# tingiskhan/pyfilter

Measured on AMD Instinct MI355X. Metric: particle-steps/sec (batch x particles x T), 1M-particle APF, higher is better.
Workload: dtype f32; 1 GPU; apf_lgo_1m: APF + lgo proposal, systematic resampling, N=1048576 particles x B=1 filters per GPU, T=250, state dim 1; parallelism=single GPU

## Files before the change

### include/pf_amd.h

```cpp
#ifndef PF_AMD_H
#define PF_AMD_H

#include <stddef.h>
#include <stdint.h>

#ifdef __cplusplus
extern "C" {
#endif

#define PF_ABI_VERSION 4

#define PF_OK 0
#define PF_EINVAL (-1)
#define PF_EWORKSPACE (-2)
#define PF_EUNSUPPORTED (-3)

#define PF_F32 0
#define PF_F64 1

#define PF_HID_LINEAR 0
#define PF_HID_SINE_EM 1
#define PF_HID_VERHULST_EM 2
#define PF_HID_LORENZ63_EM 3
#define PF_HID_OU 4
// ... 55 lines not shown

int pf_pre_weight(const pf_model* model, int proposal, const void* x, const void* y, int64_t y_rows, void* out,
                  int64_t N, int64_t B, int dtype, void* stream);

int pf_sample_and_weight(const pf_model* model, int proposal, int weigh, const void* x, const void* y,
                         int64_t y_rows, const void* z, uint64_t seed, uint32_t step, void* x_out, void* w_out,
                         int64_t N, int64_t B, int dtype, void* stream);

#define PF_NESTED_MAX 256
int pf_nested_sample_and_weight(const pf_model* model, int num_samples, const void* x, const void* y, int64_t y_rows,
                                const void* z, const void* v, uint64_t seed, uint32_t step, void* x_out, void* w_out,
                                int32_t* pick_out, int64_t N, int64_t B, int dtype, void* stream);

int pf_forecast_workspace_bytes(int64_t N, int64_t B, int steps, size_t* bytes);
int pf_forecast(const pf_model* model, int steps, const void* x, const void* W, const void* z, const void* e, uint64_t seed,
                void* x_mean, void* x_var, void* y_mean, void* y_var, void* x_path, void* y_path, void* ws, size_t ws_bytes,
                int64_t N, int64_t B, int dtype, void* stream);

int pf_initial_sample(const double* m0, const double* s0, const void* z, uint64_t seed, void* x, int64_t N,
                      int64_t B, int64_t D, int dtype, void* stream);

int pf_initial_sample_cols(const void* m0, int64_t m0_stride_b, int64_t m0_stride_d, const void* s0, int64_t s0_stride_b,
                           int64_t s0_stride_d, const void* z, uint64_t seed, void* x, int64_t N, int64_t B, int64_t D,
                           int dtype, void* stream);

int pf_observed_flags(const void* y, int64_t steps, int64_t row_elems, int dtype, uint8_t* out, void* stream);

int pf_theta_ess(const void* logw, int64_t rows, int64_t B, int dtype, void* out, void* stream);

#define PF_THETA_MAXP 8
#define PF_PRIOR_NORMAL 0
#define PF_PRIOR_LOGNORMAL 1
#define PF_PRIOR_EXPONENTIAL 2
#define PF_PRIOR_GAMMA 3
#define PF_PRIOR_HALFNORMAL 4
#define PF_PRIOR_BETA 5
#define PF_PRIOR_UNIFORM 6
typedef struct pf_theta_priors {
    int32_t P;
    int32_t kind[PF_THETA_MAXP];
    double a[PF_THETA_MAXP], b[PF_THETA_MAXP];
} pf_theta_priors;

int pf_theta_fit(const void* values, const void* logw, int64_t B, int32_t P, double scale, int dtype, void* mean, void* chol,
                 void* stream);

int pf_theta_propose(const pf_theta_priors* priors, const void* mean, const void* chol, const void* eps, int64_t B, int dtype,
                     void* u_out, void* const* x_out, void* prior_out, void* stream);

int pf_theta_accept(const void* u_cur, const void* u_star, const void* mean_f, const void* chol_f, const void* mean_r,
                    const void* chol_r, const void* prior_cur, const void* prior_star, const void* ll_cur, const void* ll_star,
                    const void* unif, int64_t B, int32_t P, int dtype, void* log_acc, uint8_t* accepted, void* rate, void* stream);

int pf_theta_path(const void* w0, const void* ll, int64_t n, int64_t B, int dtype, void* w_path, void* stats, void* host_rows,
                  uint64_t seq, const int32_t* status, void* stream);

int pf_theta_step(void* w, const void* ll, int64_t B, int dtype, void* stats, void* host_slot, uint64_t seq, void* acc,
                  const int32_t* status, void* stream);

int pf_host_alloc(size_t bytes, void** out);
int pf_host_free(void* p);

int pf_theta_resample(const void* logw, int64_t B, double u, int dtype, int64_t* ancestors, void* cdf_scratch, void* stream);

#define PF_JITTER_NONSHRINKING 0
#define PF_JITTER_SHRINKING 1
#define PF_JITTER_LIUWEST 2
#define PF_JITTER_CONSTANT 3
#define PF_JITTER_MAXB 8192

int pf_jitter_fit(const void* values, const void* logw, int64_t B, int32_t P, int32_t kind, double par, const void* scale,
                  double min_std, double bw_lo, double bw_hi, int dtype, double* fit, void* mean, void* scale_out, void* stream);

int pf_jitter_apply(const pf_theta_priors* priors, const void* values, const int64_t* ancestors, const double* fit, int64_t B,
                    int32_t kind, double par, double bw_lo, double bw_hi, int32_t discrete, const void* eps, const void* select,
                    uint64_t seed, uint64_t counter, int dtype, void* u_out, void* const* x_out, void* stream);

#define PF_ROUTE_AUTO 0
#define PF_ROUTE_PER_STEP 1
#define PF_ROUTE_COLUMN_GENERIC 2
#define PF_ROUTE_CLUSTER 3
#define PF_ROUTE_CLUSTER_ALWAYS 4
#define PF_ROUTE_CLUSTER_SPREAD 5
typedef struct pf_run_hints {
    int32_t route;
    int32_t column_max_n;
    int32_t tile_target;
    int32_t ancestor_search;
    int32_t resume;
    int32_t prepare_next;
    int32_t cluster_generation;
    int32_t cluster_patience;
} pf_run_hints;

typedef struct pf_filter_args {
    uint64_t struct_size;
    pf_model model;
    int32_t filter;
    int32_t proposal;
    int32_t resampler;
    int32_t dtype;
    int64_t N, B;
    double ess_threshold;
    uint64_t seed;
    void* x[2];
    void* logw[2];
    int32_t* anc;
    void* cdf;
    void* pos;
    const void* y;
    int64_t y_rows;
    const uint8_t* observed;
    const void* z_tape;
    const void* u_tape;
    void* means;
    void* vars;
    void* ll_steps;
    void* ll_total;
    int32_t* step_counter;
    void* ws;
    size_t ws_bytes;
    const uint8_t* observed_dev;
    int64_t ring;
    const void* user_loc;
    const void* user_scale;
    int64_t user_scale_per_column;
    double user_dt;
    int32_t* status;
    pf_run_hints hints;
} pf_filter_args;

int pf_filter_run(const pf_filter_args* args, int64_t t0, int64_t n_steps, int finalize, void* stream);

int pf_filter_observe(const pf_filter_args* args, int64_t t0, int64_t n_steps, int finalize, void* w, const void* ll, void* stats,
                      void* host_slot, uint64_t seq, void* acc, void* stream);

int pf_filter_graph_create(const pf_filter_args* args, int64_t t0, int64_t n_steps, int finalize, void* stream,
                           void** handle);
int pf_filter_graph_launch(void* handle, void* stream);
int pf_filter_graph_destroy(void* handle);

int pf_filter_run_timed(const pf_filter_args* args, int64_t t0, int64_t n_steps, int finalize, void* stream,
                        float* kernel_ms);


int pf_smooth_fixed_lag(const void* x_hist, const int32_t* anc_hist, void* out, int64_t S, int64_t N, int64_t B,
                        int64_t D, int dtype, void* stream);

int pf_smooth_ffbs(const pf_model* model, const void* x_hist, const void* logw_hist, const void* x_last, const void* u,
                   uint64_t seed, void* out, int64_t S, int64_t N, int64_t B, int dtype, void* stream);


int pf_debug_draw_normals(uint64_t seed, uint32_t step0, int64_t n_steps, void* out, int64_t N, int64_t B, int64_t D,
                          int dtype, void* stream);

int pf_debug_launch_trace(int32_t* out, int max_records);

#ifdef __cplusplus
}
#endif
#endif
```

### pyfilter_amd/_lib.py

```python
import ctypes as C
import os
from typing import Optional

import torch

_HERE = os.path.dirname(os.path.abspath(__file__))
LIB_PATH = os.path.join(_HERE, "libpfamd.so")

PF_F32, PF_F64 = 0, 1
HID_LINEAR, HID_SINE_EM, HID_VERHULST_EM, HID_LORENZ63_EM, HID_OU, HID_USER_AFFINE, HID_LINEAR_MAT = 0, 1, 2, 3, 4, 5, 6
OBS_LINEAR, OBS_SV = 0, 1
PROP_BOOTSTRAP, PROP_LGO = 0, 1
FILTER_SISR, FILTER_APF = 0, 1
RESAMPLE_SYSTEMATIC, RESAMPLE_MULTINOMIAL = 0, 1
MAX_D = 3
MAX_O = 3
LIN_MAX_D = 8
LIN_MAX_O = 8
NESTED_MAX = 256

EXPORTS = (
    "pf_version", "pf_abi_version", "pf_error_string", "pf_workspace_bytes", "pf_normalize", "pf_systematic", "pf_systematic_cdf_free", "pf_systematic_logw",
    "pf_multinomial", "pf_gather", "pf_loglik", "pf_moments", "pf_pre_weight", "pf_sample_and_weight",
    "pf_initial_sample", "pf_filter_run", "pf_filter_run_timed", "pf_filter_graph_create", "pf_filter_graph_launch",
    "pf_filter_graph_destroy", "pf_columns_gather", "pf_columns_exchange", "pf_debug_draw_normals", "pf_debug_launch_trace",
    "pf_smooth_fixed_lag", "pf_smooth_ffbs", "pf_observed_flags", "pf_theta_ess", "pf_theta_fit", "pf_theta_propose",
    "pf_theta_accept", "pf_theta_path", "pf_theta_resample", "pf_initial_sample_cols", "pf_theta_step", "pf_host_alloc",
    "pf_host_free", "pf_filter_observe", "pf_jitter_fit", "pf_jitter_apply", "pf_nested_sample_and_weight",
    "pf_forecast", "pf_forecast_workspace_bytes",
)


THETA_MAXP = 8
JITTER_NONSHRINKING, JITTER_SHRINKING, JITTER_LIUWEST, JITTER_CONSTANT = 0, 1, 2, 3
JITTER_MAXB = 8192


class PfThetaPriors(C.Structure):
    _fields_ = [("P", C.c_int32), ("kind", C.c_int32 * THETA_MAXP), ("a", C.c_double * THETA_MAXP), ("b", C.c_double * THETA_MAXP)]


class PfModel(C.Structure):
    _fields_ = [
        ("hid_kind", C.c_int32), ("obs_kind", C.c_int32), ("dim", C.c_int32), ("obs_dim", C.c_int32),
        ("dt", C.c_double), ("inc_scale", C.c_double), ("params", C.c_void_p),
    ]


ABI_VERSION = 4


class PfRunHints(C.Structure):
    _fields_ = [("route", C.c_int32), ("column_max_n", C.c_int32), ("tile_target", C.c_int32), ("ancestor_search", C.c_int32),
                ("resume", C.c_int32), ("prepare_next", C.c_int32), ("cluster_generation", C.c_int32), ("cluster_patience", C.c_int32)]


class PfFilterArgs(C.Structure):

    _fields_ = [
        ("struct_size", C.c_uint64),
        ("model", PfModel),
        ("filter", C.c_int32), ("proposal", C.c_int32), ("resampler", C.c_int32), ("dtype", C.c_int32),
        ("N", C.c_int64), ("B", C.c_int64),
        ("ess_threshold", C.c_double),
        ("seed", C.c_uint64),
        ("x", C.c_void_p * 2), ("logw", C.c_void_p * 2),
        ("anc", C.c_void_p), ("cdf", C.c_void_p), ("pos", C.c_void_p),
        ("y", C.c_void_p), ("y_rows", C.c_int64), ("observed", C.c_void_p),
        ("z_tape", C.c_void_p), ("u_tape", C.c_void_p),
        ("means", C.c_void_p), ("vars", C.c_void_p), ("ll_steps", C.c_void_p), ("ll_total", C.c_void_p),
        ("step_counter", C.c_void_p),
        ("ws", C.c_void_p), ("ws_bytes", C.c_size_t),
        ("observed_dev", C.c_void_p),
        ("ring", C.c_int64),
        ("user_loc", C.c_void_p), ("user_scale", C.c_void_p), ("user_scale_per_column", C.c_int64),
        ("user_dt", C.c_double),
        ("status", C.c_void_p),
        ("hints", PfRunHints),
    ]

    def __init__(self, *args, **kwargs):
        super().__init__(*args, **kwargs)
        self.struct_size = C.sizeof(PfFilterArgs)


_lib = None


class PfAmdError(RuntimeError):
    pass


def load() -> C.CDLL:
    global _lib
    if _lib is not None:
        return _lib
    path = LIB_PATH
    if not os.path.exists(path):
        raise PfAmdError(
            f"{path} not found: build it with `python -c 'import __graft_entry__ as g; g.build()'` "
            "(hipcc --offload-arch=gfx950).  pyfilter_amd has no CPU / eager fallback."
        )
    lib = C.CDLL(path)
    lib.pf_version.restype = C.c_char_p
    lib.pf_error_string.restype = C.c_char_p
    lib.pf_error_string.argtypes = [C.c_int]
    vp, i64, i32, u64, u32, sz = C.c_void_p, C.c_int64, C.c_int, C.c_uint64, C.c_uint32, C.c_size_t
    lib.pf_workspace_bytes.argtypes = [i64, i64, i64, C.POINTER(sz)]
    lib.pf_normalize.argtypes = [vp, vp, vp, vp, i64, i64, i32, vp, sz, vp]
    lib.pf_systematic.argtypes = [vp, vp, i32, vp, vp, vp, i64, i64, i32, vp, sz, vp]
    lib.pf_systematic_logw.argtypes = [vp, vp, i32, vp, vp, vp, i64, i64, i32, vp, sz, vp]
    lib.pf_systematic_cdf_free.argtypes = [i64, i64, i32, i32, C.POINTER(C.c_int)]
    lib.pf_multinomial.argtypes = [vp, vp, u64, u32, vp, vp, vp, i64, i64, i32, vp, sz, vp]
    lib.pf_gather.argtypes = [vp, vp, vp, vp, i64, i64, i64, i32, vp]
    lib.pf_loglik.argtypes = [vp, vp, vp, i64, i64, i32, vp, sz, vp]
    lib.pf_columns_gather.argtypes = [vp, vp, vp, i64, i64, i64, i32, vp]
    lib.pf_columns_exchange.argtypes = [vp, vp, vp, i64, i64, i64, i32, vp]
    lib.pf_moments.argtypes = [vp, vp, vp, vp, i64, i64, i64, i32, vp, sz, vp]
    lib.pf_pre_weight.argtypes = [C.POINTER(PfModel), i32, vp, vp, i64, vp, i64, i64, i32, vp]
    lib.pf_sample_and_weight.argtypes = [C.POINTER(PfModel), i32, i32, vp, vp, i64, vp, u64, u32, vp, vp, i64, i64, i32, vp]
    lib.pf_nested_sample_and_weight.argtypes = [C.POINTER(PfModel), i32, vp, vp, i64, vp, vp, u64, u32, vp, vp, vp, i64, i64, i32, vp]
    lib.pf_forecast_workspace_bytes.argtypes = [i64, i64, i32, C.POINTER(sz)]
    lib.pf_forecast.argtypes = [C.POINTER(PfModel), i32, vp, vp, vp, vp, u64, vp, vp, vp, vp, vp, vp, vp, sz, i64, i64, i32, vp]
    lib.pf_initial_sample.argtypes = [C.POINTER(C.c_double), C.POINTER(C.c_double), vp, u64, vp, i64, i64, i64, i32, vp]
    lib.pf_filter_run.argtypes = [C.POINTER(PfFilterArgs), i64, i64, i32, vp]
    lib.pf_filter_run_timed.argtypes = [C.POINTER(PfFilterArgs), i64, i64, i32, vp, C.POINTER(C.c_float)]
    lib.pf_filter_graph_create.argtypes = [C.POINTER(PfFilterArgs), i64, i64, i32, vp, C.POINTER(vp)]
    lib.pf_filter_graph_launch.argtypes = [vp, vp]
    lib.pf_filter_graph_destroy.argtypes = [vp]
    lib.pf_smooth_fixed_lag.argtypes = [vp, vp, vp, i64, i64, i64, i64, i32, vp]
    lib.pf_smooth_ffbs.argtypes = [C.POINTER(PfModel), vp, vp, vp, vp, u64, vp, i64, i64, i64, i32, vp]
    lib.pf_observed_flags.argtypes = [vp, i64, i64, i32, vp, vp]
    lib.pf_theta_ess.argtypes = [vp, i64, i64, i32, vp, vp]
    lib.pf_theta_path.argtypes = [vp, vp, i64, i64, i32, vp, vp, vp, u64, vp, vp]
    lib.pf_theta_resample.argtypes = [vp, i64, C.c_double, i32, vp, vp, vp]
    lib.pf_theta_step.argtypes = [vp, vp, i64, i32, vp, vp, u64, vp, vp, vp]
    lib.pf_filter_observe.argtypes = [C.POINTER(PfFilterArgs), i64, i64, i32, vp, vp, vp, vp, u64, vp, vp]
    lib.pf_host_alloc.argtypes = [sz, C.POINTER(vp)]
    lib.pf_host_free.argtypes = [vp]
    lib.pf_initial_sample_cols.argtypes = [vp, i64, i64, vp, i64, i64, vp, u64, vp, i64, i64, i64, i32, vp]
    lib.pf_theta_fit.argtypes = [vp, vp, i64, i32, C.c_double, i32, vp, vp, vp]
    lib.pf_theta_propose.argtypes = [C.POINTER(PfThetaPriors), vp, vp, vp, i64, i32, vp, C.POINTER(vp), vp, vp]
    lib.pf_theta_accept.argtypes = [vp] * 11 + [i64, i32, i32, vp, vp, vp, vp]
    dbl = C.c_double
    lib.pf_jitter_fit.argtypes = [vp, vp, i64, i32, i32, dbl, vp, dbl, dbl, dbl, i32, vp, vp, vp, vp]
    lib.pf_jitter_apply.argtypes = [C.POINTER(PfThetaPriors), vp, vp, vp, i64, i32, dbl, dbl, dbl, i32, vp, vp, u64, u64, i32, vp,
                                    C.POINTER(vp), vp]
    lib.pf_debug_draw_normals.argtypes = [u64, u32, i64, vp, i64, i64, i64, i32, vp]
    lib.pf_debug_launch_trace.argtypes = [C.POINTER(C.c_int32), i32]
    for name in EXPORTS:
        fn = getattr(lib, name)
        if name not in ("pf_version", "pf_error_string"):
            fn.restype = C.c_int
    if lib.pf_abi_version() != ABI_VERSION:
        raise PfAmdError(f"{path} implements ABI {lib.pf_abi_version()}, this package speaks ABI {ABI_VERSION}: rebuild it "
                         "(python -c 'import __graft_entry__ as g; g.build()')")
    _lib = lib
    return lib


def version() -> str:
    return load().pf_version().decode()


def check(rc: int, what: str):
    if rc != 0:
        raise PfAmdError(f"{what} failed: {load().pf_error_string(rc).decode()} (code {rc})")


def dtype_code(dtype: torch.dtype) -> int:
    if dtype == torch.float32:
        return PF_F32
    if dtype == torch.float64:
        return PF_F64
    raise PfAmdError(f"unsupported dtype {dtype}: the HIP kernels compute in float32 or float64")


def require_gpu(*tensors: Optional[torch.Tensor]):
    for t in tensors:
        if t is not None and not t.is_cuda:
            raise PfAmdError(
                "pyfilter_amd runs on MI355X only: got a CPU tensor (there is no CPU fallback; move the model / data "
                "to 'cuda')."
            )


def ptr(t: Optional[torch.Tensor]) -> Optional[int]:
    return None if t is None else t.data_ptr()


def stream_ptr() -> int:
    return torch._C._cuda_getCurrentRawStream(torch._C._cuda_getDevice())


_ws_cache = {}


def workspace(n: int, b: int, device: torch.device) -> torch.Tensor:
    key = (n, b, device.index, stream_ptr())
    ws = _ws_cache.get(key)
    nbytes = C.c_size_t(0)
    if ws is None:
        check(load().pf_workspace_bytes(n, b, 1, C.byref(nbytes)), "pf_workspace_bytes")
        ws = torch.empty(nbytes.value, dtype=torch.uint8, device=device)
        if len(_ws_cache) > 64:
            _ws_cache.clear()
        _ws_cache[key] = ws
    return ws


def new_workspace(n: int, b: int, device: torch.device) -> torch.Tensor:
    nbytes = C.c_size_t(0)
    check(load().pf_workspace_bytes(n, b, MAX_D, C.byref(nbytes)), "pf_workspace_bytes")
    return torch.zeros(nbytes.value, dtype=torch.uint8, device=device)
```

### pyfilter_amd/csrc/pf_fused.hpp

```cpp
#pragma once

namespace pf {

#define PF_STEP_B blockIdx.x
#define PF_STEP_K blockIdx.y

#ifdef PF_DEVTOOLS
#define PF_CUT(a, n) ((a).debug_cut == (n))
#define PF_STAMP(a, slot)                                                                       \
    do {                                                                                        \
        if ((a).debug_cut < 0 && !(a).finalize_only && PF_STEP_K == (unsigned)(-(a).debug_cut - 1) &&  \
            PF_STEP_B == 0 && threadIdx.x == 0)                                                 \
            (a).dbg[slot] = (unsigned long long)clock64();                                      \
    } while (0)
#else
#define PF_CUT(a, n) false
#ifdef PF_ISA_MARKS
#define PF_STAMP(a, slot) asm volatile("; PF_MARK " #slot)
#else
#define PF_STAMP(a, slot) do { } while (0)
#endif
#endif

template <typename T> struct FusedArgs {
    ModelDesc md;
    const T* params;
    int filter, proposal, resampler;
    Geom g;
    double thr_abs;
    double logN;
    T rcN;
    uint64_t seed;
    const uint64_t* seed_dev;
    T* x[2];
    T* logw[2];
    int32_t* anc;
    const int32_t* anc_prev;
    T* cdf;
    T* pos;
    const T* y;
    int y_rows;
    const T* z_tape;
    const T* u_tape;
    const T* user_loc;
    const T* user_scale;
    int user_scale_percol;
    T user_dt;
    T* means;
    T* vars;
    T* ll_steps;
    T* ll_total;
    double* part;
    int64_t part_stride;
    ColStat* stat;
    int32_t* poison;
    T* cpack;
    double* piv0;
    double* ctab;
    int64_t ctab_stride;
    int t0;
    int step;
    int obs;
    int obs_next;
    const uint8_t* obs_dev;
    __device__ __forceinline__ bool y_informative() const {
        const T* yr = y + (int64_t)step * md.obs_dim;
        bool any = false;
        for (int o = 0; o < md.obs_dim; ++o) any = any || !(yr[o] != yr[o]);
        return any;
    }
    __device__ __forceinline__ bool is_obs() const { return obs >= 0 ? obs != 0 : (obs == -1 ? obs_dev[step] != 0 : y_informative()); }
    __device__ __forceinline__ bool is_obs_next() const { return obs_next >= 0 ? obs_next != 0 : obs_dev[step + 1] != 0; }
    int finalize_only;
    int book_inline;
    unsigned kmap;
    __device__ __forceinline__ int tile_of_row(unsigned y) const {
        return (int)(((y & (kmap & 0xffu)) << ((kmap >> 8) & 0xffu)) + (y >> ((kmap >> 16) & 0xffu)));
    }
    unsigned long long* dbg;
    __device__ __forceinline__ const double* part_r() const { return part + (int64_t)(step & 1) * part_stride; }
    __device__ __forceinline__ double* part_w(int state) const { return part + (int64_t)(state & 1) * part_stride; }
    __device__ __forceinline__ const double* ctab_r(int b) const {
        return ctab + (int64_t)(step & 1) * ctab_stride + (int64_t)b * g.tiles * g.rounds_per_tile * PF_NWAVES * 2;
    }
    __device__ __forceinline__ double* ctab_w(int state, int b) const {
        return ctab + (int64_t)(state & 1) * ctab_stride + (int64_t)b * g.tiles * g.rounds_per_tile * PF_NWAVES * 2;
    }
    template <int D> __device__ __forceinline__ T pivot(int q, int b, int d) const {
        return (q - 2 >= t0) ? means[((int64_t)(q - 2) * g.B + b) * D + d] : (T)piv0[(int64_t)b * PF_MAXD + d];
    }
    int debug_cut;
    int keep_state;
};

template <typename T, int D>
__device__ __forceinline__ void load_col_params(const FusedArgs<T>& a, int b, int step, bool with_y, ColParams<T, D>& cp,
                                                int late = 0) {
    const int O = a.md.obs_dim;
    const int NP = 4 * D + O * D + 2 * O;
    cp.load(a.params + (int64_t)b * NP + late, O,
            with_y ? a.y + ((int64_t)step * a.y_rows + (a.y_rows == 1 ? 0 : b)) * O + late : nullptr);
}

template <typename T, int D, bool WQ = true> struct PartialAcc {
    T m1, m2;
    T s1, s2, q1;
    T mx[D], mxx[D];
    double es;
    bool poison;
    __device__ __forceinline__ void init() {
        m1 = m2 = -Lim<T>::inf();
        s1 = s2 = q1 = T(0);
        es = 0.0;
#pragma unroll
        for (int d = 0; d < D; ++d) mx[d] = mxx[d] = T(0);
        poison = false;
    }
    template <int VEC>
    __device__ __forceinline__ void push_round(const T (&lw)[VEC], const T (&x)[D][VEC], bool pre_on, const T (&pre)[VEC],
                                               const T (&piv)[D], T (&e_out)[VEC]) {
        T m = lw[0];
#pragma unroll
        for (int j = 1; j < VEC; ++j) m = (lw[j] > m) ? lw[j] : m;
        if (m > m1) {
            const T rs = (m1 == -Lim<T>::inf()) ? T(0) : pf_exp_w(m1 - m);
            s1 *= rs;
            if constexpr (WQ) q1 *= rs * rs;
#pragma unroll
            for (int d = 0; d < D; ++d) {
                mx[d] *= rs;
                mxx[d] *= rs;
            }
            m1 = m;
        }
#pragma unroll
        for (int j = 0; j < VEC; ++j) {
            T e = (lw[j] == -Lim<T>::inf()) ? T(0) : pf_exp_w(lw[j] - m1);
            if (lw[j] != lw[j]) e = lw[j];
            e_out[j] = e;
            s1 += e;
            if constexpr (WQ) q1 += e * e;
#pragma unroll
            for (int d = 0; d < D; ++d) {
                const T xd = x[d][j] - piv[d];
                mx[d] += e * xd;
                mxx[d] += e * xd * xd;
            }
        }
        if (pre_on) {
            T rw[VEC];
#pragma unroll
            for (int j = 0; j < VEC; ++j) {
                if (is_nan_or_posinf(pre[j])) poison = true;
                rw[j] = sanitize_logw(pre[j] + lw[j]);
            }
            T mm = rw[0];
#pragma unroll
            for (int j = 1; j < VEC; ++j) mm = (rw[j] > mm) ? rw[j] : mm;
            if (mm > m2) {
                s2 *= (m2 == -Lim<T>::inf()) ? T(0) : pf_exp_w(m2 - mm);
                m2 = mm;
            }
#pragma unroll
            for (int j = 0; j < VEC; ++j) {
                const T e = (rw[j] == -Lim<T>::inf()) ? T(0) : pf_exp_w(rw[j] - m2);
                e_out[j] = e;
                s2 += e;
            }
        }
    }
    template <bool WITH_ES, typename FB, typename FA>
    __device__ __forceinline__ void finish(double* part, int b, int k, int B, int tiles, bool pre_on, double* red, T* redm,
                                           int32_t* poison_slot, T& M1_out, T& M2_out, T& F1_out, T& F2_out, FB&& before, FA&& after) {
        const int lane = threadIdx.x & 63, wid = threadIdx.x >> 6;
        const T w1 = wave_max<T>(m1), w2 = wave_max<T>(m2);
        if (lane == 0) {
            redm[wid] = w1;
// ... 520 lines not shown
    double mv[2 * D];
    ColPartials<true, 2 * D> p1;
    ColPartials<false, 0> p2;
    load_col_partials<true, 2 * D>(a.part_r(), stride, cb, g.tiles, PQ_M1, PQ_S1, PQ_MX, p1);
    if (two) load_col_partials<false, 0>(a.part_r(), stride, cb, g.tiles, PQ_M2, PQ_S2, 0, p2);
    const ColSums c1 = column_sums<T, true, false, 2 * D>(p1, g.tiles, nullptr, nullptr, redm, red, mv);
    ColSums c2{0.0, 1.0, 0.0};
    if (two) c2 = column_sums<T, false, false>(p2, g.tiles, nullptr, nullptr, redm, red);
    const double lse_w = c1.M + log(c1.S);
    const double ess = c1.S * c1.S / c1.Q;
    bool resample = apf ? obs : (ess < a.thr_abs);
    if (a.finalize_only) resample = false;
    if (threadIdx.x == 0) {
#pragma unroll
        for (int d = 0; d < D; ++d) {
            const double dm = mv[d] / c1.S;
            double var = mv[D + d] / c1.S - dm * dm;
            if (var < 0.0) var = 0.0;
            a.means[((int64_t)step * g.B + b) * D + d] = (T)(piv[d] + dm);
            a.vars[((int64_t)step * g.B + b) * D + d] = (T)var;
        }
        if (step > 0 && !st.ll_done) {
            double ll = 0.0;
            if (st.prev_observed) {
                ll = lse_w - st.base_lse;
                if (poisoned) ll = __builtin_nan("");
            }
            a.poison[pslot * g.B + b] = 0;
            a.ll_steps[(int64_t)(step - 1) * g.B + b] = (T)ll;
            a.ll_total[b] = (T)(ll_tot + ll);
        }
        st.lse_w = lse_w;
        if (!a.finalize_only) st.resample = resample ? 1 : 0;
        st.ll_done = a.finalize_only ? 1 : 0;
        if (!a.finalize_only) {
            st.prev_observed = obs ? 1 : 0;
            st.base_lse = apf ? a.logN - ((c2.M + log(c2.S)) - lse_w) : (resample ? a.logN : lse_w);
        }
        a.stat[b] = st;
    }
}

template <typename T, int D>
__global__ __launch_bounds__(PF_BLOCK) void k_fused_book(FusedArgs<T> a) {
    __shared__ double red[(2 + 2 * D) * PF_NWAVES];
    __shared__ double redm[PF_NWAVES];
    column_bookkeeping<T, D>(a, blockIdx.y, red, redm);
}

#define PF_WAVES_D1_GENERIC 4
#define PF_WAVES_D1_MN 3
#define PF_WAVES_DN_A 3
template <typename T, int D, int MODE, int PROP, bool FAST, int SPEC, bool MULTI> struct StepWaves {
    static constexpr int value = sizeof(T) != 4 ? 1
                                 : (D == 1 && MODE == 1 && MULTI) ? PF_WAVES_D1_MN
                                 : D == 1     ? (FAST ? 4 : PF_WAVES_D1_GENERIC)
                                 : PROP == PF_PROP_LGO ? 2
                                 : (MODE == 1 || SPEC == 2) ? PF_WAVES_DN_A
                                 : 3;
};
template <typename T, int D, int VEC> struct StepShared {
    static constexpr int WIN = SearchWin<T, VEC>::WIN;
    static constexpr bool XWIN = (sizeof(T) * D <= 8);
    T* win;
    T* xwin;
    int* sh_j0;
    int* sh_cl;
    int* sh_wm;
    double* red;
    double* reds;
    T* redm;
    double* ptl;
    double* ftl;
    int* sh_plan;
    double* crec;
};
template <typename T> struct StepPlan {
    int j0, kt0;
    T ub;
    double offE, invE;
    bool resample;
    bool have_z0;
};
template <typename T, int D, int VEC, int MODE, int SPEC, bool EARLY_Z, bool MULTI>
__device__ __forceinline__ StepPlan<T> step_prologue(const FusedArgs<T>& a, const StepShared<T, D, VEC>& sh, T (&z0)[VEC][D]) {
    const Geom& g = a.g;
    const int b = PF_STEP_B, k = a.tile_of_row(PF_STEP_K);
    const int step = a.step;
    const bool obs = SPEC ? true : a.is_obs();
    const bool apf = SPEC ? (SPEC == 1) : (a.filter == PF_FILTER_APF);
    const bool two = apf && obs;
    StepPlan<T> pl{0, 0, T(0), 0.0, 0.0, false, false};
    PF_STAMP(a, 0);
#ifdef PF_DEVTOOLS
    if (a.debug_cut < 0 && threadIdx.x == 0 && b == 0 && (k % 128) == 0 && k / 128 < 8) a.dbg[16 + k / 128] = wall_clock64();
#endif
    if (apf && !obs) return pl;
    constexpr bool multinomial = MODE == 1;
    const uint64_t seed = a.seed + (a.seed_dev ? *a.seed_dev : 0ull);
    const T u_taped = (!multinomial && a.u_tape) ? a.u_tape[(int64_t)step * g.B + b] : T(0);
    const int64_t stride = (int64_t)g.B * g.tiles;
    const int64_t cb = (int64_t)b * g.tiles;
    double* const redm_d = sh.red + 2 * PF_NWAVES;
    T e0[1] = {T(0)};
    if constexpr (multinomial) {
        T tail[1];
        draw_exponentials<T, 1>(seed, PF_STREAM_MULTINOMIAL, (uint32_t)step, (uint64_t)((int64_t)g.B * g.N + b), tail);
        spacing_table(a.part_r(), stride, cb, g.tiles, (double)tail[0], sh.ptl, sh.reds);
        pl.offE = sh.ptl[k];
        pl.invE = 1.0 / sh.ptl[g.tiles + 1];
        draw_exponentials<T, 1>(seed, PF_STREAM_MULTINOMIAL, (uint32_t)step, (uint64_t)((int64_t)b * g.N + (int64_t)k * g.tile_elems), e0);
    }
    ColPartials<true, 0> p1;
    ColPartials<false, 0> p2;
    constexpr bool SHORT = MULTI;
    const bool one_tile = SHORT && g.tiles == 1 && a.debug_cut != 77;
    double m1 = 0.0, s1 = 0.0, q1 = 0.0;
    if (one_tile) {
        const double* part = a.part_r();
        m1 = part[(two ? PQ_M2 : PQ_M1) * stride + cb];
        s1 = part[(two ? PQ_S2 : PQ_S1) * stride + cb];
        q1 = two ? 0.0 : part[PQ_Q1 * stride + cb];
    }
    const bool few_tiles = SHORT && !one_tile && g.tiles <= PF_WAVE && a.debug_cut != 79;
    if (!one_tile && !few_tiles) {
        if (two) load_col_partials<false, 0>(a.part_r(), stride, cb, g.tiles, PQ_M2, PQ_S2, 0, p2);
        else load_col_partials<true, 0>(a.part_r(), stride, cb, g.tiles, PQ_M1, PQ_S1, 0, p1);
    }
    if (EARLY_Z && (SPEC || !a.z_tape)) {
        const int64_t i0 = (int64_t)k * g.tile_elems + threadIdx.x * VEC;
        if (i0 < g.N) draw_normals<T, D, VEC>(seed, PF_STREAM_NORMAL, (uint32_t)step, (uint64_t)((int64_t)b * g.N + i0), z0);
        pl.have_z0 = true;
    }
    if (one_tile) {
        if (two) {
            column_sums_one_tile<T, false>(m1, s1, q1, sh.ptl, sh.ftl);
            pl.resample = true;
        } else {
            const ColSums c = column_sums_one_tile<T, true>(m1, s1, q1, sh.ptl, sh.ftl);
            pl.resample = c.S * c.S / c.Q < a.thr_abs;
        }
    } else if (few_tiles) {
        if (two) {
            column_sums_wave<T, false>(a.part_r(), stride, cb, g.tiles, PQ_M2, PQ_S2, sh.ptl, sh.ftl);
            pl.resample = true;
        } else {
            const ColSums c = column_sums_wave<T, true>(a.part_r(), stride, cb, g.tiles, PQ_M1, PQ_S1, sh.ptl, sh.ftl);
            pl.resample = c.S * c.S / c.Q < a.thr_abs;
        }
    } else if (two) {
        column_sums<T, false, true>(p2, g.tiles, sh.ptl, sh.ftl, redm_d, sh.red);
        pl.resample = true;
    } else {
        const ColSums c = column_sums<T, true, true>(p1, g.tiles, sh.ptl, sh.ftl, redm_d, sh.red);
        pl.resample = c.S * c.S / c.Q < a.thr_abs;
    }
    PF_STAMP(a, 1);
    if (!pl.resample) return pl;
    const double* ptl = sh.ptl;
    T p;
    if constexpr (multinomial) {
        p = (T)((pl.offE + (double)e0[0]) * pl.invE);
    } else {
        pl.ub = a.u_tape ? u_taped : uniform_draw<T>(seed, PF_STREAM_UNIFORM, (uint32_t)step, (uint64_t)b);
        p = grid_position<T>((int64_t)k * g.tile_elems, pl.ub, T(g.N));
    }
    if (one_tile && a.debug_cut != 78) {
        pl.j0 = 0;
        pl.kt0 = 0;
        return pl;
    }
    if (threadIdx.x < PF_WAVE) {
        const int lane = threadIdx.x;
        int lo = 0, hi = g.tiles - 1;
        while (lo < hi) {
            const int len = hi - lo + 1;
            const int st = (len + PF_WAVE - 1) / PF_WAVE;
            int probe = lo + (lane + 1) * st - 1;
            if (probe > hi) probe = hi;
            const bool ge = (probe >= g.tiles - 1) || !((T)ptl[probe + 1] < p);
            const unsigned long long bal = __ballot(ge);
            const int f = bal ? __ffsll((long long)bal) - 1 : PF_WAVE - 1;
            int nhi = lo + (f + 1) * st - 1;
            if (nhi > hi) nhi = hi;
            lo = lo + f * st;
            if (lo > nhi) lo = nhi;
            hi = nhi;
        }
        const int kt = lo;
        const double Pk = ptl[kt], Pn = ptl[kt + 1], fk = sh.ftl[kt];
        const int64_t first = (int64_t)kt * g.tile_elems;
        const int64_t last = (first + g.tile_elems < g.N ? first + g.tile_elems : g.N) - 1;
        const T* l_col = ((step & 1) ? a.pos : a.cdf) + (int64_t)b * g.N;
        const int64_t len = last + 1 - first;
        auto cdf_at = [&](int64_t q) -> T {
            if constexpr (MULTI) {
                const double* cg = a.ctab_r(b) + 2 * (q / (PF_WAVE * VEC));
                return cdf_from_local<T>(l_col[q], cg[0], cg[1], Pk, fk, Pn, q == last, q == g.N - 1);
            } else {
                return cdf_from_local<T>(l_col[q], Pk, fk, Pn, q == last, q == g.N - 1);
            }
        };
        int64_t res;
        bool found;
        {
            float fr = (float)((double)p - Pk) * __builtin_amdgcn_rcpf((float)(Pn - Pk));
            fr = __builtin_fminf(__builtin_fmaxf(fr, 0.0f), 1.0f);
            int64_t g0 = first + (int64_t)(fr * (float)len) - (PF_WAVE / 2) * PF_PROBE_STEP;
            const int64_t g0max = last - (PF_WAVE - 1) * PF_PROBE_STEP;
            if (g0 > g0max) g0 = g0max;
            if (g0 < first) g0 = first;
            int64_t q = g0 + (int64_t)lane * PF_PROBE_STEP;
            if (q > last) q = last;
            const unsigned long long bal = __ballot(cdf_at(q) >= p);
            const int f = bal ? __ffsll((long long)bal) - 1 : 0;
            found = bal != 0 && (f > 0 || g0 == first);
            res = f > 0 ? g0 + (int64_t)(f - 1) * PF_PROBE_STEP + 1 : first;
        }
        if (!found) {
            const int64_t st = (len + PF_WAVE - 1) / PF_WAVE;
            int64_t probe = first + (lane + 1) * st - 1;
            if (probe > last) probe = last;
            const unsigned long long bal = __ballot(cdf_at(probe) >= p);
            const int f = bal ? __ffsll((long long)bal) - 1 : PF_WAVE - 1;
            res = first + (int64_t)f * st;
            if (res > last) res = last;
        }
        if (lane == 0) {
            sh.sh_plan[0] = (int)res;
            sh.sh_plan[1] = kt;
        }
    }
    __syncthreads();
    pl.j0 = sh.sh_plan[0];
    pl.kt0 = sh.sh_plan[1];
    PF_STAMP(a, 2);
    return pl;
}
template <typename T, int D, int VEC, int MODE, int PROP, bool FAST, int SPEC, int MK, bool RS, bool MULTI>
__device__ __forceinline__ void step_body(const FusedArgs<T>& a, const StepShared<T, D, VEC>& sh, const StepPlan<T>& pl,
                                          const T (&z0)[VEC][D]) {
    const int proposal = (PROP >= 0) ? PROP : a.proposal;
    ModelDesc md = a.md;
    if constexpr (!FAST && MK == 1) { md.hid_kind = PF_HID_VERHULST_EM; md.obs_kind = PF_OBS_SV; md.obs_dim = 1; }
    if constexpr (!FAST && MK == 4) { md.hid_kind = PF_HID_LORENZ63_EM; md.obs_kind = PF_OBS_LINEAR; }
    constexpr bool USER = !FAST && MK == 3;
    constexpr int WIN = StepShared<T, D, VEC>::WIN;
    constexpr int V1 = (MODE == 0) ? 1 : VEC;
    constexpr int STAGED = PF_BLOCK * (VEC + V1);
    constexpr bool XWIN = StepShared<T, D, VEC>::XWIN;
    T* const win = sh.win;
    T* const xwin = sh.xwin;
    int& sh_j0 = *sh.sh_j0;
    int* const sh_cl = sh.sh_cl;
    int* const sh_wm = sh.sh_wm;
    double* const red = sh.red;
    double* const reds = sh.reds;
    T* const redm = sh.redm;
    int* hd = reinterpret_cast<int*>(win);
    const Geom& g = a.g;
    const int b = PF_STEP_B, k = a.tile_of_row(PF_STEP_K);
    const int tid = threadIdx.x;
    const int step = a.step;
    const int slot = step & 1;
    const bool obs = SPEC ? true : a.is_obs();
    const bool apf = SPEC ? (SPEC == 1) : (a.filter == PF_FILTER_APF);
    constexpr bool resample = RS;
    constexpr bool multinomial = MODE == 1;
    const bool windowed = resample;
    const bool pre_next = SPEC ? (SPEC == 1) : (a.is_obs_next() && apf);
    const int N = (int)g.N;
    PF_STAMP(a, 8);
    if (PF_CUT(a, 1)) return;

    int j0 = pl.j0;
    int kt0 = pl.kt0;
    const double offE = pl.offE, invE = pl.invE;
    double carryE = 0.0;
    const uint64_t seed = a.seed + (a.seed_dev ? *a.seed_dev : 0ull);
    const T* z_step = (!SPEC && a.z_tape) ? a.z_tape + (int64_t)step * D * g.B * g.N : nullptr;

    ColParams<T, D> cp;
    ColConsts<T, D> cc;
    FastCol<T> fc;
    if constexpr (!FAST && D > 1) {
        load_col_params<T, D>(a, b, step, obs, cp);
        if (pre_next) cp.load_next(a.y + ((int64_t)(step + 1) * a.y_rows + (a.y_rows == 1 ? 0 : b)) * a.md.obs_dim);
    }
    const T ub = pl.ub;

    const T* x_in = a.x[slot];
    const T* lw_in = a.logw[slot] + (int64_t)b * g.N;
#ifdef PF_DEVTOOLS
    T* lw_out = a.logw[slot ^ 1] + (int64_t)b * g.N;
    int32_t* anc_col = a.anc + (int64_t)b * g.N;
#endif
    const T* cdf_col = ((step & 1) ? a.pos : a.cdf) + (int64_t)b * g.N;
    const int64_t base = (int64_t)k * g.tile_elems;
    const T nT = T(N);
    const T rcN = a.rcN;
    const bool pow2 = (N & (N - 1)) == 0;

    bool poison = false;
    PartialAcc<T, D, SPEC != 1> acc;
    acc.init();
    PF_STAMP(a, 9);
    const double* ptab_col = sh.ptl;
    const double* ftab_col = sh.ftl;
    CdfView<T> view;
    view.L = cdf_col;
    view.ptab = ptab_col;
    view.ftab = ftab_col;
    const double* const ct_col = MULTI ? a.ctab_r(b) : nullptr;
    view.ct = ct_col;
    view.chunk_elems = PF_WAVE * VEC;
    view.N = N;
    view.tile_elems = g.tile_elems;
    view.tiles = g.tiles;

    T e_rw[VEC];
    T rwn[VEC];
#pragma unroll
    for (int j = 0; j < VEC; ++j) {
        e_rw[j] = T(0);
        rwn[j] = -Lim<T>::inf();
    }
    const bool scan_next = !apf || pre_next;
    constexpr bool single = !MULTI;
    const bool use_lds = g.rounds_per_tile * PF_NWAVES <= PF_LDS_CHUNKS;
    double* const ct_tile = a.ctab_w(step + 1, b) + 2 * (int64_t)k * g.rounds_per_tile * PF_NWAVES;
    T* const l_next = ((step & 1) ? a.cdf : a.pos) + (int64_t)b * g.N;
    int rk = 0;
    for (int r = 0; r < g.rounds_per_tile; ++r) {
        const int64_t r0 = base + (int64_t)r * g.round_elems;
        if (r0 >= g.N) break;
        const int64_t i0 = r0 + tid * VEC;
        const bool on = i0 < g.N;
        if (MODE == 0 && windowed) {
            int zero[VEC];
#pragma unroll
            for (int j = 0; j < VEC; ++j) zero[j] = 0;
            if (VEC == 1) hd[tid] = 0; else store_vec<int, VEC>(hd + tid * VEC, zero);
        }
        T pv[VEC];
        if (multinomial && windowed) {
            T ev[VEC];
            double incl[VEC], local = 0.0, total;
            if (on) draw_exponentials<T, VEC>(seed, PF_STREAM_MULTINOMIAL, (uint32_t)step, (uint64_t)((int64_t)b * g.N + i0), ev);
#pragma unroll
            for (int j = 0; j < VEC; ++j) {
                local += on ? (double)ev[j] : 0.0;
                incl[j] = local;
            }
            const double excl = block_scan_excl(local, reds, total);
#pragma unroll
            for (int j = 0; j < VEC; ++j) pv[j] = (T)((offE + carryE + excl + incl[j]) * invE);
            carryE += total;
        }

        const int ws = j0 - (j0 % VEC);
        T c0[VEC], c1[V1], xa[D][VEC], xb[D][V1];
        const int ja = ws + tid * VEC, jb = ws + PF_BLOCK * VEC + tid * V1;
        const bool ina = windowed && ja < N, inb = windowed && jb < N;
        if (ina) {
            if (VEC == 1) c0[0] = cdf_col[ja]; else load_vec<T, VEC>(cdf_col + ja, c0);
            if (XWIN) {
#pragma unroll
                for (int d = 0; d < D; ++d) {
                    const T* xc = x_in + ((int64_t)d * g.B + b) * g.N + ja;
                    if (VEC == 1) xa[d][0] = xc[0]; else load_vec<T, VEC>(xc, xa[d]);
                }
            }
        }
        if (inb) {
            if (V1 == 1) c1[0] = cdf_col[jb]; else load_vec<T, V1>(cdf_col + jb, c1);
            if (XWIN) {
#pragma unroll
                for (int d = 0; d < D; ++d) {
                    const T* xc = x_in + ((int64_t)d * g.B + b) * g.N + jb;
                    if (V1 == 1) xb[d][0] = xc[0]; else load_vec<T, V1>(xc, xb[d]);
                }
            }
        }
        T lw_old[VEC];
        if (on && !resample) {
            if (VEC == 1) lw_old[0] = lw_in[i0]; else load_vec<T, VEC>(lw_in + i0, lw_old);
        }

        T zt[VEC][D];
        if (on) {
            if (z_step) {
#pragma unroll
                for (int d = 0; d < D; ++d) {
                    T zr[VEC];
                    const T* zc = z_step + ((int64_t)d * g.B + b) * g.N + i0;
                    if (VEC == 1) zr[0] = zc[0]; else load_vec<T, VEC>(zc, zr);
#pragma unroll
                    for (int j = 0; j < VEC; ++j) zt[j][d] = zr[j];
                }
            } else if (r == 0 && pl.have_z0) {
#pragma unroll
                for (int j = 0; j < VEC; ++j)
#pragma unroll
                    for (int d = 0; d < D; ++d) zt[j][d] = z0[j][d];
            } else {
                draw_normals<T, D, VEC>(seed, PF_STREAM_NORMAL, (uint32_t)step, (uint64_t)((int64_t)b * g.N + i0), zt);
            }
        }
        PF_STAMP(a, 10);
#ifdef PF_DEVTOOLS
        if (PF_CUT(a, 4)) {
            if (on) lw_out[i0] = zt[0][0] + zt[VEC - 1][D - 1];
            continue;
        }
// ... 18 lines not shown
                const int la = (int)(ea < (unsigned)N ? ea : (unsigned)N) - 1;
                const int lb = (int)(eb < (unsigned)N ? eb : (unsigned)N) - 1;
                if constexpr (MULTI) {
                    const double* cga = ct_col + 2 * ((wina ? wja : 0) / (PF_WAVE * VEC));
                    const double* cgb = ct_col + 2 * ((winb ? wjb : 0) / (PF_WAVE * VEC));
                    const double Ca = cga[0], ga = cga[1], Cb = cgb[0], gb = cgb[1];
#pragma unroll
                    for (int j = 0; j < VEC; ++j) {
                        const bool tl = (j == VEC - 1) && (wja + j == la);
                        m0[j] = wina ? cdf_from_local<T>(m0[j], Ca, ga, tPa, tFa, tNa, tl, tl && (wja + j == N - 1)) : Lim<T>::inf();
                    }
#pragma unroll
                    for (int j = 0; j < V1; ++j)
                        m1[j] = winb ? cdf_from_local<T>(m1[j], Cb, gb, tPb, tFb, tNb, wjb + j == lb, wjb + j == N - 1) : Lim<T>::inf();
                } else {
#pragma unroll
                    for (int j = 0; j < VEC; ++j) {
                        const bool tl = (j == VEC - 1) && (wja + j == la);
                        m0[j] = wina ? cdf_from_local<T>(m0[j], tPa, tFa, tNa, tl, tl && (wja + j == N - 1)) : Lim<T>::inf();
                    }
#pragma unroll
                    for (int j = 0; j < V1; ++j)
                        m1[j] = winb ? cdf_from_local<T>(m1[j], tPb, tFb, tNb, wjb + j == lb, wjb + j == N - 1) : Lim<T>::inf();
                }
            };
            map_window(ws, ja, jb, ina, inb, c0, c1);
            if (XWIN) {
#pragma unroll
                for (int d = 0; d < D; ++d) {
                    if (ina) { if (VEC == 1) xwin[d * WIN + tid] = xa[d][0]; else store_vec<T, VEC>(xwin + d * WIN + tid * VEC, xa[d]); }
                    if (inb) { if (V1 == 1) xwin[d * WIN + PF_BLOCK * VEC + tid] = xb[d][0]; else store_vec<T, V1>(xwin + d * WIN + PF_BLOCK * VEC + tid * V1, xb[d]); }
                }
            }
            if constexpr (MODE != 0) {
                if (VEC == 1) { win[tid] = c0[0]; win[PF_BLOCK + tid] = c1[0]; }
                else { store_vec<T, VEC>(win + tid * VEC, c0); store_vec<T, VEC>(win + (PF_BLOCK + tid) * VEC, c1); }
                __syncthreads();
                T pp[VEC];
                int qq[VEC];
#pragma unroll
                for (int j = 0; j < VEC; ++j) pp[j] = multinomial ? pv[j] : grid_position<T>(i0 + j, ub, nT);
                window_lower_bound_flat<T, WIN, VEC>(win, pp, qq);
#pragma unroll
                for (int j = 0; j < VEC; ++j) {
                    const int64_t i = i0 + j;
                    int res = N - 1;
                    if (i < N) {
                        res = (qq[j] < WIN) ? ws + qq[j] : view.lower_bound(ws + WIN < N ? ws + WIN : N, pp[j], kt0);
                        if (res > N - 1) res = N - 1;
                    }
                    idx[j] = res;
                }
            } else {
                inverse_grid_round<T, VEC, V1>(c0, c1, ws, (int)r0, g.round_elems, N, ub, nT, rcN, pow2, i0, hd, sh_cl, sh_wm,
                                           [&](int it, T (&d0)[VEC], T (&d1)[V1]) -> bool {
                                               const int w0 = ws + it * STAGED;
                                               if (w0 >= N) return false;
                                               const int wja = w0 + tid * VEC, wjb = w0 + PF_BLOCK * VEC + tid * V1;
                                               const bool wina = wja < N, winb = wjb < N;
                                               if (wina) { if (VEC == 1) d0[0] = cdf_col[wja]; else load_vec<T, VEC>(cdf_col + wja, d0); }
                                               if (winb) { if (V1 == 1) d1[0] = cdf_col[wjb]; else load_vec<T, V1>(cdf_col + wjb, d1); }
                                               map_window(w0, wja, wjb, wina, winb, d0, d1);
                                               return true;
                                           },
                                           [&](int64_t i, int from) { return view.lower_bound(from, grid_position<T>(i, ub, nT), from ? kt0 : 0); },
                                           idx);
            }
            if (r + 1 < g.rounds_per_tile) {
                if (tid == PF_BLOCK - 1) sh_j0 = idx[VEC - 1];
                __syncthreads();
                j0 = sh_j0;
            }
        } else {
#pragma unroll
            for (int j = 0; j < VEC; ++j) idx[j] = (int)((i0 + j < g.N) ? (i0 + j) : (g.N - 1));
        }
        PF_STAMP(a, 11);
#ifdef PF_DEVTOOLS
        if (on && PF_CUT(a, 2)) {
            if (VEC == 1) anc_col[i0] = idx[0]; else store_vec<int, VEC>(anc_col + i0, idx);
        }
#endif

        int late;
        asm volatile("v_readfirstlane_b32 %0, %1\n\ts_and_b32 %0, %0, 0" : "=s"(late) : "v"(idx[0]) : "scc");
        using KArgs = const __attribute__((address_space(4))) FusedArgs<T>;
        KArgs* la = (KArgs*)((const_ptr<char>)__builtin_amdgcn_kernarg_segment_ptr() + late);
        T* const x_out = la->x[slot ^ 1];
        if constexpr (FAST) {
            const_ptr<T> yq = (const_ptr<T>)(uintptr_t)a.y + late;
            const int yc = a.y_rows == 1 ? 0 : b;
            const T y_t = obs ? yq[(int64_t)step * a.y_rows + yc] : T(0);
            const T y_n = pre_next ? yq[(int64_t)(step + 1) * a.y_rows + yc] : T(0);
            fc.load((const_ptr<T>)(uintptr_t)(a.cpack + (int64_t)b * PK_N) + late, y_t, y_n);
        } else if constexpr (D == 1) {
            load_col_params<T, D>(a, b, step, obs, cp, late);
            if (pre_next) cp.load_next(a.y + ((int64_t)(step + 1) * a.y_rows + (a.y_rows == 1 ? 0 : b)) * a.md.obs_dim + late);
            cc.prepare(md, cp);
            if constexpr (USER) {
                if (la->user_scale_percol) cc.prepare_user(md, cp, la->user_scale[b]);
            } else {
                __builtin_assume(cc.fast == FAST);
            }
        } else if (r == 0) {
            cc.prepare(md, cp);
            __builtin_assume(cc.fast == FAST);
        }
        T xo[D][VEC];
        if (on && !PF_CUT(a, 2)) {
            T lwo[VEC], pre_n[VEC];
            T xr[VEC][D];
            if (!resample) {
#pragma unroll
                for (int d = 0; d < D; ++d) {
                    T xv[VEC];
                    const T* xc = x_in + ((int64_t)d * g.B + b) * g.N + i0;
                    if (VEC == 1) xv[0] = xc[0]; else load_vec<T, VEC>(xc, xv);
#pragma unroll
                    for (int j = 0; j < VEC; ++j) xr[j][d] = xv[j];
                }
            } else {
#pragma unroll
                for (int j = 0; j < VEC; ++j) {
                    const int q = idx[j] - ws;
                    const bool in_lds = XWIN && windowed && q >= 0 && q < STAGED;
#pragma unroll
                    for (int d = 0; d < D; ++d)
                        xr[j][d] = in_lds ? xwin[d * WIN + q] : x_in[((int64_t)d * g.B + b) * g.N + idx[j]];
                }
            }
#pragma unroll
            for (int j = 0; j < VEC; ++j) {
                T xn[D];
                T w_new;
                UserMS<T, D> um = UserMS<T, D>::none();
                if constexpr (USER) {
                    um.gather(la->user_loc, la->user_scale, (int64_t)b * g.N, (int64_t)g.B * g.N, idx[j], la->user_scale_percol != 0, b, g.B);
                    um.euler(xr[j], la->user_dt);
                }
                if (obs) {
                    T wi, pre_anc = T(0);
                    if constexpr (FAST) {
                        if (apf) wi = fc.template sample_and_weight_apf<FAST ? MK : 0>(proposal, xr[j][0], zt[j][0], xn[0], pre_anc);
                        else wi = fc.template sample_and_weight<FAST ? MK : 0>(proposal, xr[j][0], zt[j][0], xn[0]);
                    } else {
                        wi = sample_and_weight<T, D>(md, proposal, cp, cc, xr[j], zt[j], xn, um);
                    }
                    if (apf) {
                        if constexpr (FAST) w_new = wi - pre_anc;
                        else w_new = wi - pre_weight<T, D>(md, proposal, cp, cc, xr[j], false, um);
                        if (is_nan_or_posinf(w_new)) poison = true;
                    } else {
                        if (is_nan_or_posinf(wi)) poison = true;
                        w_new = resample ? wi : (wi + lw_old[j]);
                    }
                } else {
                    if constexpr (FAST) fc.template sample_and_weight<FAST ? MK : 0>(PF_PROP_BOOTSTRAP, xr[j][0], zt[j][0], xn[0]);
                    else sample_and_weight<T, D>(md, PF_PROP_BOOTSTRAP, cp, cc, xr[j], zt[j], xn, um);
                    w_new = resample ? T(0) : lw_old[j];
                }
                lwo[j] = sanitize_logw(w_new);
#pragma unroll
                for (int d = 0; d < D; ++d) xo[d][j] = xn[d];
                if constexpr (FAST) pre_n[j] = pre_next ? fc.template pre_weight<FAST ? MK : 0>(proposal, xn[0], true) : T(0);
                else if constexpr (USER) {
                    pre_n[j] = pre_next ? pre_weight<T, D>(md, proposal, cp, cc, xn, true, um) : T(0);
                } else pre_n[j] = pre_next ? pre_weight<T, D>(md, proposal, cp, cc, xn, true) : T(0);
                if (j & 1) __builtin_amdgcn_sched_barrier(0);
            }
            PF_STAMP(a, 12);
            const bool keep = la->keep_state != 0;
            const bool st_anc = keep || !apf;
            const bool st_lw = keep || !(apf && obs && pre_next);
#pragma unroll
            for (int d = 0; d < D; ++d) {
                T* xc = x_out + ((int64_t)d * g.B + b) * g.N + r0;
                if (VEC == 1) xc[tid] = xo[d][0]; else store_out<T, VEC, !MULTI>(xc, tid * VEC, xo[d]);
            }
            if (st_lw) {
                T* const lw_st = la->logw[slot ^ 1] + (int64_t)b * g.N;
                if (VEC == 1) lw_st[i0] = lwo[0]; else store_out<T, VEC, !MULTI>(lw_st + r0, tid * VEC, lwo);
            }
            if (resample || apf) {
                if (st_anc) {
                    int32_t* const anc_st = la->anc + (int64_t)b * g.N;
                    if (VEC == 1) anc_st[i0] = idx[0]; else store_out<int, VEC, !MULTI>(anc_st + r0, tid * VEC, idx);
                }
            } else if (la->anc_prev) {
                const int32_t* ap = la->anc_prev + (int64_t)b * g.N + i0;
                int32_t* const anc_st = la->anc + (int64_t)b * g.N;
                int prev[VEC];
                if (VEC == 1) prev[0] = ap[0]; else load_vec<int, VEC>(ap, prev);
                if (VEC == 1) anc_st[i0] = prev[0]; else store_vec<int, VEC>(anc_st + i0, prev);
            }
#ifdef PF_DEVTOOLS
            if (PF_CUT(a, 5)) {
                if (pre_next) { if (VEC == 1) lw_out[i0] = pre_n[0]; else store_vec<T, VEC>(lw_out + i0, pre_n); }
                continue;
            }
#endif
            T piv[D];
#pragma unroll
            for (int d = 0; d < D; ++d)
                piv[d] = (step - 1 >= a.t0) ? la->means[((int64_t)(step - 1) * g.B + b) * D + d] : (T)la->piv0[(int64_t)b * PF_MAXD + d];
            if constexpr (MULTI) {
#pragma unroll
                for (int j = 0; j < VEC; ++j) {
                    if (pre_next && is_nan_or_posinf(pre_n[j])) acc.poison = true;
                    rwn[j] = pre_next ? sanitize_logw(pre_n[j] + lwo[j]) : lwo[j];
                }
            }
            acc.template push_round<VEC>(lwo, xo, single && pre_next, pre_n, piv, e_rw);
            if (multinomial) {
                T ev[VEC];
                draw_exponentials<T, VEC>(seed, PF_STREAM_MULTINOMIAL, (uint32_t)(step + 1), (uint64_t)((int64_t)b * g.N + i0), ev);
#pragma unroll
                for (int j = 0; j < VEC; ++j) acc.es += (double)ev[j];
            }
            PF_STAMP(a, 13);
        }
        if (scan_next && !single) {
            chunk_scan_round<T, VEC, false>(rwn, on, l_next + r0, tid * VEC, r * PF_NWAVES + (tid >> 6), use_lds ? sh.crec : nullptr, ct_tile);
#pragma unroll
            for (int j = 0; j < VEC; ++j) rwn[j] = -Lim<T>::inf();
            ++rk;
        }
        if (windowed && r + 1 < g.rounds_per_tile) __syncthreads();
    }
    if (poison) atomicOr(&a.poison[(step & 3) * g.B + b], 1);
    if (PF_CUT(a, 3)) return;
    PF_STAMP(a, 14);
    T M1, M2, F1, F2;
    constexpr bool fused_tail = single && MODE != 1 && VEC == 4;
    const bool tile_scan = scan_next && fused_tail;
    const int64_t i0s = base + tid * VEC;
    const bool on_s = i0s < g.N;
    double e[VEC], local = 0.0, incl = 0.0;
    acc.template finish<MODE == 1>(a.part_w(step + 1), b, k, g.B, g.tiles, single && pre_next, red, redm, &a.poison[((step + 1) & 3) * g.B + b], M1, M2, F1, F2,
        [&](T f1, T f2) {
            if (!tile_scan) return;
            const T f = pre_next ? f2 : f1;
#pragma unroll
            for (int j = 0; j < VEC; ++j) {
                local += on_s ? (double)(e_rw[j] * f) : 0.0;
                e[j] = local;
            }
            incl = wave_scan_incl(local, tid & 63);
            if ((tid & 63) == 63) reds[tid >> 6] = incl;
        },
        [&]() {
            if (!tile_scan) return;
            double wave_off = 0.0;
#pragma unroll
            for (int w = 0; w < PF_NWAVES; ++w) {
                const double sw = reds[w];
                if (w < (tid >> 6)) wave_off += sw;
            }
            const double excl = wave_off + incl - local;
            if (on_s) {
                T outv[VEC];
#pragma unroll
                for (int j = 0; j < VEC; ++j) outv[j] = (T)(excl + e[j]);
                if (VEC == 1) l_next[i0s] = outv[0]; else store_out<T, VEC, !MULTI>(l_next + base, tid * VEC, outv);
            }
        });
    if (PF_CUT(a, 6)) return;
    if (scan_next && single && !fused_tail) {
        const T f = pre_next ? F2 : F1;
        double total;
#pragma unroll
        for (int j = 0; j < VEC; ++j) {
            local += on_s ? (double)(e_rw[j] * f) : 0.0;
            e[j] = local;
        }
        const double excl = block_scan_excl(local, reds, total);
        if (on_s) {
            T outv[VEC];
#pragma unroll
            for (int j = 0; j < VEC; ++j) outv[j] = (T)(excl + e[j]);
            if (VEC == 1) l_next[i0s] = outv[0]; else store_out<T, VEC, !MULTI>(l_next + base, tid * VEC, outv);
        }
    } else if (scan_next && !single) {
        double Mc, Sc;
        finalize_chunk_table<T>(ct_tile, use_lds ? sh.crec : nullptr, rk * PF_NWAVES, reds, redm, Mc, Sc);
        if (tid == 0) {
            const int64_t stride = (int64_t)g.B * g.tiles, o = (int64_t)b * g.tiles + k;
            if (pre_next) {
                a.part_w(step + 1)[PQ_M2 * stride + o] = Mc;
                a.part_w(step + 1)[PQ_S2 * stride + o] = Sc;
            } else {
                a.part_w(step + 1)[PQ_S1 * stride + o] = Sc;
            }
        }
    }
    PF_STAMP(a, 15);
#ifdef PF_DEVTOOLS
    if (a.debug_cut < 0 && tid == 0 && b == 0 && (k % 128) == 0 && k / 128 < 8) a.dbg[24 + k / 128] = wall_clock64();
#endif
}

template <typename T, int D, int VEC, int MODE, int PROP, bool FAST, int SPEC, int MK, bool MULTI>
__global__ __launch_bounds__(PF_BLOCK, (StepWaves<T, D, MODE, PROP, FAST, SPEC, MULTI>::value)) void k_fused_step(FusedArgs<T> a) {
    using SH = StepShared<T, D, VEC>;
    __shared__ __attribute__((aligned(32))) T win[SH::WIN];
    __shared__ __attribute__((aligned(32))) T xwin[SH::XWIN ? D * SH::WIN : VEC];
    __shared__ int sh_j0;
    __shared__ int sh_cl[2 * PF_NWAVES], sh_wm[PF_NWAVES];
    __shared__ double red[(4 + 2 * D) * PF_NWAVES];
    __shared__ double reds[PF_NWAVES];
    __shared__ T redm[2 * PF_NWAVES];
    __shared__ double ptl[PF_MAX_TILES + 2], ftl[PF_MAX_TILES];
    __shared__ int sh_plan[2];
    __shared__ double crec[MULTI ? 2 * PF_LDS_CHUNKS : 2];
    __shared__ double redb[PF_NWAVES];
    if (!a.book_inline && PF_STEP_K == (unsigned)a.g.tiles) {
        column_bookkeeping<T, D>(a, PF_STEP_B, red, redb);
        return;
    }
    const SH sh{win, xwin, &sh_j0, sh_cl, sh_wm, red, reds, redm, ptl, ftl, sh_plan, crec};
    T z0[VEC][D];
#pragma unroll
    for (int j = 0; j < VEC; ++j)
#pragma unroll
        for (int d = 0; d < D; ++d) z0[j][d] = T(0);
    const StepPlan<T> pl = step_prologue<T, D, VEC, MODE, SPEC, (FAST && D == 1 && sizeof(T) == 4), MULTI>(a, sh, z0);
    if constexpr (SPEC == 1) {
        step_body<T, D, VEC, MODE, PROP, FAST, SPEC, MK, true, MULTI>(a, sh, pl, z0);
    } else {
        if (pl.resample) step_body<T, D, VEC, MODE, PROP, FAST, SPEC, MK, true, MULTI>(a, sh, pl, z0);
        else step_body<T, D, VEC, MODE, PROP, FAST, SPEC, MK, false, MULTI>(a, sh, pl, z0);
    }
    if (a.book_inline == 1 && PF_STEP_K == (unsigned)a.g.tiles - 1u)
        column_bookkeeping<T, D>(a, PF_STEP_B, red, redb);
}

template <typename W> __global__ __launch_bounds__(PF_BLOCK) void k_zero_words(W* __restrict__ p, size_t n) {
    const size_t i = (size_t)blockIdx.x * PF_BLOCK + threadIdx.x;
    if (i < n) p[i] = W(0);
}

template <typename T>
__global__ __launch_bounds__(PF_WAVE) void k_observed_flags(const T* __restrict__ y, int64_t row_elems, uint8_t* __restrict__ out) {
    const T* row = y + (int64_t)blockIdx.x * row_elems;
    bool any = false;
    for (int64_t i = threadIdx.x; i < row_elems; i += PF_WAVE) any |= !(row[i] != row[i]);
    const unsigned long long bal = __ballot(any);
    if (threadIdx.x == 0) out[blockIdx.x] = bal ? 1 : 0;
}

template <typename T>
__global__ __launch_bounds__(PF_BLOCK) void k_zero_and_flags(uint32_t* __restrict__ p, size_t n, unsigned zero_blocks, const T* __restrict__ y,
                                                             int64_t row_elems, uint8_t* __restrict__ out) {
    if (blockIdx.x < zero_blocks) {
        const size_t i = (size_t)blockIdx.x * PF_BLOCK + threadIdx.x;
        if (i < n) p[i] = 0u;
        return;
    }
    if (threadIdx.x >= PF_WAVE) return;
    const unsigned k = blockIdx.x - zero_blocks;
    const T* row = y + (int64_t)k * row_elems;
    bool any = false;
    for (int64_t i = threadIdx.x; i < row_elems; i += PF_WAVE) any |= !(row[i] != row[i]);
    const unsigned long long bal = __ballot(any);
    if (threadIdx.x == 0) out[k] = bal ? 1 : 0;
}

template <typename T>
__device__ __forceinline__ void theta_ess_row(const T* w, int64_t B, T* out, T* redm, double* red) {
    T m = -Lim<T>::inf();
    bool finite = true;
    for (int64_t i = threadIdx.x; i < B; i += PF_BLOCK) {
        const T v = w[i];
        finite &= !(is_nan_or_posinf(v) || v == -Lim<T>::inf());
        const T s = is_nan_or_posinf(v) ? -Lim<T>::inf() : v;
        m = s > m ? s : m;
    }
    m = block_max<T>(m, redm);
    double acc[3] = {0.0, 0.0, finite ? 0.0 : 1.0};
    if (m > -Lim<T>::inf()) {
        for (int64_t i = threadIdx.x; i < B; i += PF_BLOCK) {
            const T v = w[i];
            const double e = is_nan_or_posinf(v) ? 0.0 : exp((double)v - (double)m);
            acc[0] += e;
            acc[1] += e * e;
        }
    }
    block_sum<3>(acc, red);
    if (threadIdx.x == 0) {
        out[0] = (T)(acc[1] > 0.0 ? acc[0] * acc[0] / acc[1] : (double)B);
        out[1] = acc[2] == 0.0 ? T(1) : T(0);
    }
}
template <typename T>
__global__ __launch_bounds__(PF_BLOCK) void k_theta_ess(const T* __restrict__ w, int64_t B, T* __restrict__ out) {
    __shared__ T redm[PF_NWAVES];
    __shared__ double red[3 * PF_NWAVES];
    theta_ess_row<T>(w + (int64_t)blockIdx.x * B, B, out + 2 * (int64_t)blockIdx.x, redm, red);
// ... 4 lines not shown
```

### pyfilter_amd/csrc/pf_host.hpp

```cpp
#pragma once
#include <hip/hip_runtime.h>
#include <stdint.h>

#include <atomic>
#include <cstdlib>
#include <cstring>
#include <mutex>
#include <vector>

#include <type_traits>

#include "../../include/pf_amd.h"
#include "pf_device.hpp"
#include "pf_models.hpp"
#include "pf_philox.hpp"
#include "pf_linear.hpp"

namespace pf {

#define PF_MAX_TILES 1024
#define PF_TARGET_WGS 1024
#define PF_AUTO_FLAGS 128

struct Geom {
// ... 125 lines not shown
}

enum { PQ_M1 = 0, PQ_S1 = 1, PQ_Q1 = 2, PQ_M2 = 3, PQ_S2 = 4, PQ_E = 5, PQ_MX = 6 };

}

#include "pf_search.hpp"
#include "pf_fused.hpp"
#include "pf_column.hpp"
#include "pf_cluster.hpp"

namespace pf {
struct ThetaFold {
    void* w;
    const void* ll;
    void* stats;
    void* slot;
    uint64_t seq;
    void* acc;
    int folded;
};
}

using namespace pf;

static inline int launch_status() {
    const hipError_t e = hipGetLastError();
    return e == hipSuccess ? PF_OK : (int)e;
}
#define PF_CHECK_LAUNCH()                          \
    do {                                           \
        if (const int e_ = launch_status()) return e_; \
    } while (0)

template <int V> using int_c = std::integral_constant<int, V>;
template <typename F> static inline int with_dtype(int dtype, F&& f) {
    if (dtype == PF_F32) return f(float{});
    if (dtype == PF_F64) return f(double{});
    return PF_EINVAL;
}
template <typename F> static inline int with_vec(int vec, F&& f) { return vec == 4 ? f(int_c<4>{}) : f(int_c<1>{}); }
template <typename F> static inline int with_d3(int64_t D, F&& f) {
    return D == 1 ? f(int_c<1>{}) : D == 2 ? f(int_c<2>{}) : f(int_c<3>{});
}
template <typename F> static inline int with_d8(int64_t D, F&& f) {
    switch (D) {
        case 1: return f(int_c<1>{}); case 2: return f(int_c<2>{}); case 3: return f(int_c<3>{}); case 4: return f(int_c<4>{});
        case 5: return f(int_c<5>{}); case 6: return f(int_c<6>{}); case 7: return f(int_c<7>{}); case 8: return f(int_c<8>{});
        default: return PF_EUNSUPPORTED;
    }
}
template <typename F> static inline int with_bool(bool b, F&& f) { return b ? f(std::true_type{}) : f(std::false_type{}); }

static inline bool bad_shape(int64_t N, int64_t B) { return N < 1 || B < 1 || N > (int64_t)1 << 30 || B > 65535; }

static inline int check_model(const pf_model* m, bool fused = false) {
    if (!m || !m->params) return PF_EINVAL;
    if (m->hid_kind == PF_HID_USER_AFFINE && !fused) return PF_EUNSUPPORTED;
    if (m->hid_kind == PF_HID_LINEAR_MAT) {
        if (fused || m->dim < 1 || m->dim > PF_LIN_MAXD || m->obs_dim < 1 || m->obs_dim > PF_LIN_MAXO || m->obs_kind != PF_OBS_LINEAR)
            return PF_EUNSUPPORTED;
        return PF_OK;
    }
    if (m->dim < 1 || m->dim > PF_MAXD || m->obs_dim < 1 || m->obs_dim > PF_MAXO) return PF_EUNSUPPORTED;
    if (m->dim == 1 && m->obs_dim != 1) return PF_EUNSUPPORTED;
    if (m->hid_kind < 0 || m->hid_kind > PF_HID_USER_AFFINE) return PF_EUNSUPPORTED;
    if (m->hid_kind == PF_HID_LORENZ63_EM && m->dim != 3) return PF_EUNSUPPORTED;
    if (m->obs_kind != PF_OBS_LINEAR && m->obs_kind != PF_OBS_SV) return PF_EUNSUPPORTED;
    if (m->obs_kind == PF_OBS_SV && m->dim != 1) return PF_EUNSUPPORTED;
    return PF_OK;
}

static inline ModelDesc to_desc(const pf_model* m) {
    ModelDesc d;
    d.hid_kind = m->hid_kind;
    d.obs_kind = m->obs_kind;
    d.obs_dim = m->obs_dim;
    d.dt = m->dt;
    d.inc_scale = m->inc_scale;
    return d;
}

#define PF_TRACE_LEN 2048
#define PF_TRACE_FIELDS 10
struct LaunchTrace {
    int32_t rec[PF_TRACE_LEN][PF_TRACE_FIELDS];
    uint64_t count;
};
LaunchTrace& launch_trace();
static inline void trace_launch(int step, int tbytes, int d, int vec, int mode, int prop, int fast, int spec, int mk, int multi) {
    LaunchTrace& t = launch_trace();
    int32_t* r = t.rec[t.count % PF_TRACE_LEN];
    r[0] = step; r[1] = tbytes; r[2] = d; r[3] = vec; r[4] = mode; r[5] = prop; r[6] = fast; r[7] = spec; r[8] = mk; r[9] = multi;
    ++t.count;
}

template <typename T>
static FusedArgs<T> make_fused_args(const pf_filter_args* A, const Geom& g, const WsLayout& wl, int64_t t0) {
    FusedArgs<T> a;
    a.md = to_desc(&A->model);
    a.params = (const T*)A->model.params;
    a.filter = A->filter;
    a.proposal = A->proposal;
    a.resampler = A->resampler;
    a.g = g;
    a.thr_abs = A->ess_threshold * (double)A->N;
    a.logN = log((double)A->N);
    a.rcN = T(1) / T(A->N);
    a.seed = A->seed;
    a.seed_dev = (const uint64_t*)A->step_counter;
    a.x[0] = (T*)A->x[0];
    a.x[1] = (T*)A->x[1];
    a.logw[0] = (T*)A->logw[0];
    a.logw[1] = (T*)A->logw[1];
    a.anc = A->anc;
    a.anc_prev = nullptr;
    a.cdf = (T*)A->cdf;
    a.pos = (T*)A->pos;
    a.y = (const T*)A->y;
    a.y_rows = (int)A->y_rows;
    a.z_tape = (const T*)A->z_tape;
    a.u_tape = (const T*)A->u_tape;
    a.user_loc = (const T*)A->user_loc;
    a.user_scale = (const T*)A->user_scale;
    a.user_scale_percol = A->user_scale_per_column != 0 ? 1 : 0;
    a.user_dt = (T)A->user_dt;
    a.means = (T*)A->means;
    a.vars = (T*)A->vars;
    a.ll_steps = (T*)A->ll_steps;
    a.ll_total = (T*)A->ll_total;
    a.part = (double*)((char*)A->ws + wl.off_part);
    a.part_stride = (int64_t)wl.part_elems;
    a.stat = (ColStat*)((char*)A->ws + wl.off_stat);
    a.poison = (int32_t*)((char*)A->ws + wl.off_poison);
    a.dbg = (unsigned long long*)((char*)A->ws + wl.off_dbg);
    a.cpack = (T*)((char*)A->ws + wl.off_cpack);
    a.piv0 = (double*)((char*)A->ws + wl.off_piv0);
    a.ctab = (double*)((char*)A->ws + wl.off_ctab);
    a.ctab_stride = (int64_t)wl.ctab_elems;
    static_assert(PK_N == 24, "workspace layout reserves 24 slots per column record");
    a.finalize_only = 0;
    a.t0 = (int)t0;
    a.debug_cut = 0;
    a.keep_state = 1;
#ifdef PF_DEVTOOLS
    if (const char* dc = getenv("PF_DEBUG_CUT")) a.debug_cut = atoi(dc);
#endif
    return a;
}

template <typename T>
struct ObsFlags {
    const uint8_t* host;
    const uint8_t* dev;
    bool inline_y;
    bool derive;
    uint8_t* slot;
    int64_t row;
    const T* y;

    ObsFlags(const pf_filter_args* A, const WsLayout& wl, int64_t t0, int64_t n_steps) {
        const bool none = !A->observed && !A->observed_dev && n_steps > 0;
        host = A->observed;
        inline_y = none && n_steps == 1 && A->y_rows == 1;
        derive = none && !inline_y;
        slot = (uint8_t*)A->ws + wl.off_ctr + 64;
        row = A->y_rows * (int64_t)A->model.obs_dim;
        y = derive ? (const T*)A->y + t0 * row : nullptr;
        dev = derive ? slot - t0 : A->observed_dev;
    }
    int obs(int64_t t) const { return inline_y ? -2 : dev ? -1 : (host[t] != 0); }
    void launch_derive(int64_t n_steps, hipStream_t st) const {
        hipLaunchKernelGGL((k_observed_flags<T>), dim3((unsigned)n_steps), dim3(PF_WAVE), 0, st, y, row, slot);
    }
    void launch_zero(uint32_t* p, size_t words, bool flags, int64_t n_steps, hipStream_t st) const {
        const unsigned zb = (unsigned)((words + PF_BLOCK - 1) / PF_BLOCK);
        if (flags)
            hipLaunchKernelGGL((k_zero_and_flags<T>), dim3(zb + (unsigned)n_steps), dim3(PF_BLOCK), 0, st, p, words, zb, y, row, slot);
        else
            hipLaunchKernelGGL((k_zero_words<uint32_t>), dim3(zb), dim3(PF_BLOCK), 0, st, p, words);
    }
    ColumnRun piece(int64_t t, int64_t left) const {
        ColumnRun r;
        r.t0 = (int)t;
        r.n_steps = (int)(left < 32 * PFC_OBS_WORDS ? left : 32 * PFC_OBS_WORDS);
        r.use_bits = (dev == nullptr && !inline_y) ? 1 : 0;
        r.inline_y = inline_y ? 1 : 0;
        for (int w = 0; w < PFC_OBS_WORDS; ++w) r.obs_bits[w] = 0u;
        if (r.use_bits)
            for (int q = 0; q < r.n_steps; ++q)
                if (host[r.t0 + q]) r.obs_bits[q >> 5] |= 1u << (q & 31);
        return r;
    }
};

struct KernelTimer {
    float* kernel_ms;
    hipStream_t st;
    hipEvent_t ev[2] = {nullptr, nullptr};
    bool failed = false;
    int rc = PF_OK;
    KernelTimer(float* kernel_ms_, hipStream_t st_) : kernel_ms(kernel_ms_), st(st_) {
        if (!kernel_ms) return;
        for (auto& e : ev)
            if (hipEventCreate(&e) != hipSuccess) {
                failed = true;
                rc = (int)hipGetLastError();
                return;
            }
        (void)hipEventRecord(ev[0], st);
    }
    ~KernelTimer() {
        for (auto& e : ev)
            if (e) (void)hipEventDestroy(e);
    }
    void stop() const {
        if (kernel_ms) (void)hipEventRecord(ev[1], st);
    }
    int finish(int64_t n_steps) const {
        if (!kernel_ms) return PF_OK;
        const hipError_t se = hipStreamSynchronize(st);
        if (se != hipSuccess) return (int)se;
        float ms = 0.f;
        (void)hipEventElapsedTime(&ms, ev[0], ev[1]);
        kernel_ms[0] = kernel_ms[2] = n_steps > 0 ? ms / (float)n_steps : 0.f;
        kernel_ms[1] = 0.f;
        return PF_OK;
    }
};

template <int... KINDS, typename F>
static bool with_folded(const pf_filter_args* A, F&& f) {
    bool hit = false;
    auto with_kind = [&](auto kind_c) {
        constexpr bool SV = decltype(kind_c)::value == PF_HID_VERHULST_EM;
        if (hit || A->model.hid_kind != decltype(kind_c)::value || A->model.obs_kind != (SV ? PF_OBS_SV : PF_OBS_LINEAR)) return;
        if (A->proposal != PF_PROP_BOOTSTRAP && (SV || A->proposal != PF_PROP_LGO)) return;
        hit = true;
        auto with_prop = [&](auto filt_c) {
            if constexpr (!SV) {
                if (A->proposal == PF_PROP_LGO) return f(kind_c, filt_c, int_c<PF_PROP_LGO>{});
            }
            f(kind_c, filt_c, int_c<PF_PROP_BOOTSTRAP>{});
        };
        if (A->filter == PF_FILTER_APF) with_prop(int_c<PF_FILTER_APF>{});
        else with_prop(int_c<PF_FILTER_SISR>{});
    };
    if (!A->z_tape) (with_kind(int_c<KINDS>{}), ...);
    return hit;
}

template <typename T, int D, int VEC, bool MULTI>
int filter_run_impl(const pf_filter_args* A, const Geom& g, const WsLayout& wl, int64_t t0, int64_t n_steps, int finalize,
                    hipStream_t st, float* kernel_ms);

static inline int column_threads(int64_t N, int vec) {
    const int64_t need = (N + vec - 1) / vec;
    return (int)(((need + PF_WAVE - 1) / PF_WAVE) * PF_WAVE);
}
#define PF_COLUMN_VEC 4
static inline size_t column_lds_bytes(int64_t N, int D, size_t tsize, int vec) {
    int64_t np2 = 64;
    while (np2 < N) np2 <<= 1;
    const int64_t NP = ((N + vec - 1) / vec) * vec;
    const size_t planes = (((size_t)(np2 + PF_LB_PAD + (int64_t)D * NP) * tsize) + 15) & ~(size_t)15;
    return planes + sizeof(double) * (2 + 2 * (4 + 2 * D)) * PFC_MAXW + 16;
}
#define PF_COLUMN_MAX_N 2048
static inline bool column_eligible(const pf_filter_args* A, const Geom& g, int64_t n_steps, int finalize) {
    if (!finalize || n_steps < 1 || A->ring >= 3) return false;
    if (A->hints.route == PF_ROUTE_PER_STEP) return false;
    const int64_t max_n = A->hints.column_max_n > 0 ? A->hints.column_max_n : PF_COLUMN_MAX_N;
    if (A->N > max_n || column_threads(A->N, PF_COLUMN_VEC) > 1024) return false;
    return column_lds_bytes(A->N, A->model.dim, A->dtype == PF_F64 ? 8 : 4, PF_COLUMN_VEC) <= 64 * 1024;
}

int pf_run_column_f32(const pf_filter_args* A, const Geom& g, const WsLayout& wl, int64_t t0, int64_t n_steps, hipStream_t st, float* kernel_ms);
int pf_run_column_f64(const pf_filter_args* A, const Geom& g, const WsLayout& wl, int64_t t0, int64_t n_steps, hipStream_t st, float* kernel_ms);

#define PFK_HOST_VEC 4
#define PF_CLUSTER_INFEASIBLE (-1000)
static inline size_t cluster_lds_bytes(int D, size_t tsize) {
    return (size_t)(PFK_WIN_P2 + D * PFK_WIN) * tsize + 2 * PFK_FOLD * sizeof(double);
}
static inline bool cluster_eligible(const pf_filter_args* A, const Geom& g, int64_t n_steps, int finalize) {
    if (A->hints.route != PF_ROUTE_CLUSTER && A->hints.route != PF_ROUTE_CLUSTER_ALWAYS && A->hints.route != PF_ROUTE_CLUSTER_SPREAD) return false;
    if (!finalize || n_steps < 1 || A->ring >= 3) return false;
    if (A->N <= PF_CLUSTER_MIN_N || A->N > PF_CLUSTER_MAX_N || A->N % PFK_HOST_VEC != 0) return false;
    if (A->resampler != PF_RESAMPLE_SYSTEMATIC || A->model.hid_kind == PF_HID_USER_AFFINE) return false;
    const int64_t members = ((A->N + PFK_TPB * PFK_HOST_VEC - 1) / (PFK_TPB * PFK_HOST_VEC)) * A->B;
    if (A->hints.route == PF_ROUTE_CLUSTER && members > 2 * 1024) return false;
    (void)g;
    return true;
}
int pf_run_cluster_f32(const pf_filter_args* A, const Geom& g, const WsLayout& wl, int64_t t0, int64_t n_steps, hipStream_t st, float* kernel_ms,
                       ThetaFold* theta);
int pf_run_cluster_f64(const pf_filter_args* A, const Geom& g, const WsLayout& wl, int64_t t0, int64_t n_steps, hipStream_t st, float* kernel_ms,
                       ThetaFold* theta);
```

### pyfilter_amd/csrc/pf_kernels.hip

```cpp
#include "pf_host.hpp"

namespace pf {

template <typename T, int VEC>
__device__ __forceinline__ void systematic_round(const T* __restrict__ cdf_col, int N, int64_t i0, T u,
                                                 const T* __restrict__ u_elem, T* win, int* sh_j0, int (&idx)[VEC]) {
    constexpr int WIN = SearchWin<T, VEC>::WIN;
    const int tid = threadIdx.x;
    const int j0 = *sh_j0;
    const int ws = j0 - (j0 % VEC);
    {
        T v0[VEC], v1[VEC];
        const int ja = ws + tid * VEC, jb = ws + (PF_BLOCK + tid) * VEC;
        const bool ina = ja < N, inb = jb < N;
        if (ina) { if (VEC == 1) v0[0] = cdf_col[ja]; else load_vec<T, VEC>(cdf_col + ja, v0); }
        if (inb) { if (VEC == 1) v1[0] = cdf_col[jb]; else load_vec<T, VEC>(cdf_col + jb, v1); }
#pragma unroll
        for (int j = 0; j < VEC; ++j) {
            if (!ina) v0[j] = Lim<T>::inf();
            if (!inb) v1[j] = Lim<T>::inf();
        }
        if (VEC == 1) { win[tid] = v0[0]; win[PF_BLOCK + tid] = v1[0]; }
        else { store_vec<T, VEC>(win + tid * VEC, v0); store_vec<T, VEC>(win + (PF_BLOCK + tid) * VEC, v1); }
    }
// ... 1695 lines not shown
    JitterDraws dr;
    dr.eps = eps;
    dr.select = select;
    dr.seed = (unsigned long long)seed;
    dr.counter = (unsigned long long)counter;
    hipStream_t st = (hipStream_t)stream;
    const dim3 grid((unsigned)((B + PF_BLOCK - 1) / PF_BLOCK));
    return with_dtype(dtype, [&](auto t) {
        using T = decltype(t);
        hipLaunchKernelGGL((k_jitter_apply<T>), grid, dim3(PF_BLOCK), 0, st, pr, (const T*)values, ancestors, fit, (int)B, (int)kind, par,
                           bw_lo, bw_hi, (int)discrete, 1.0 / sqrt((double)B), dr, (T*)u_out, out);
        return launch_status();
    });
}

extern "C" int pf_theta_ess(const void* logw, int64_t rows, int64_t B, int dtype, void* out, void* stream) {
    if (!logw || !out || B < 1 || rows < 0 || rows > 0x7fffffff) return PF_EINVAL;
    if (rows == 0) return PF_OK;
    hipStream_t st = (hipStream_t)stream;
    const dim3 grid((unsigned)rows);
    return with_dtype(dtype, [&](auto t) {
        using T = decltype(t);
        hipLaunchKernelGGL((k_theta_ess<T>), grid, dim3(PF_BLOCK), 0, st, (const T*)logw, B, (T*)out);
        return launch_status();
    });
}



extern "C" int pf_smooth_fixed_lag(const void* x_hist, const int32_t* anc_hist, void* out, int64_t S, int64_t N, int64_t B,
                                   int64_t D, int dtype, void* stream) {
    if (!x_hist || !anc_hist || !out || S < 1 || bad_shape(N, B) || D < 1) return PF_EINVAL;
    const dim3 grid(ew_blocks(N), (int)B);
    hipStream_t st = (hipStream_t)stream;
    return with_dtype(dtype, [&](auto t) {
        using T = decltype(t);
        hipLaunchKernelGGL((k_trace_ancestors<T>), grid, dim3(PF_BLOCK), 0, st, (const T*)x_hist, anc_hist, (T*)out, S, N, (int)B, (int)D);
        return launch_status();
    });
}

extern "C" int pf_smooth_ffbs(const pf_model* model, const void* x_hist, const void* logw_hist, const void* x_last,
                              const void* u, uint64_t seed, void* out, int64_t S, int64_t N, int64_t B, int dtype,
                              void* stream) {
    if (!model || !x_hist || !logw_hist || !x_last || !out || S < 1 || bad_shape(N, B)) return PF_EINVAL;
    int rc = check_model(model);
    if (rc) return rc;
    if (model->hid_kind == PF_HID_LINEAR_MAT) return PF_EUNSUPPORTED;
    const ModelDesc md = to_desc(model);
    const dim3 grid((unsigned)((N + PF_BLOCK - 1) / PF_BLOCK), (int)B);
    hipStream_t st = (hipStream_t)stream;
    return with_dtype(dtype, [&](auto t) {
        return with_d3(model->dim, [&](auto d) {
            using T = decltype(t);
            hipLaunchKernelGGL((k_ffbs<T, decltype(d)::value>), grid, dim3(PF_BLOCK), 0, st, md, (const T*)model->params, (const T*)x_hist,
                               (const T*)logw_hist, (const T*)x_last, (const T*)u, seed, (T*)out, S, N, (int)B);
            return launch_status();
        });
    });
}

extern "C" int pf_debug_draw_normals(uint64_t seed, uint32_t step0, int64_t n_steps, void* out, int64_t N, int64_t B,
                                     int64_t D, int dtype, void* stream) {
    if (!out || bad_shape(N, B) || D < 1 || D > PF_MAXD || n_steps < 1 || n_steps > 65535) return PF_EINVAL;
    const Geom g = make_geom(N, B);
    const dim3 grid((unsigned)((N + g.round_elems - 1) / g.round_elems), (unsigned)B, (unsigned)n_steps);
    hipStream_t st = (hipStream_t)stream;
    return with_dtype(dtype, [&](auto t) {
        return with_vec(g.vec, [&](auto v) {
            return with_d3(D, [&](auto d) {
                using T = decltype(t);
                hipLaunchKernelGGL((k_debug_normals<T, decltype(d)::value, decltype(v)::value>), grid, dim3(PF_BLOCK), 0, st, seed, step0,
                                   (T*)out, N, (int)B);
                return launch_status();
            });
        });
    });
}

LaunchTrace& launch_trace() {
    static thread_local LaunchTrace t = {};
    return t;
}
extern "C" int pf_debug_launch_trace(int32_t* out, int max_records) {
    if (!out || max_records < 0) return PF_EINVAL;
    const LaunchTrace& t = launch_trace();
    const uint64_t have = t.count < PF_TRACE_LEN ? t.count : PF_TRACE_LEN;
    const int n = (uint64_t)max_records < have ? max_records : (int)have;
    for (int i = 0; i < n; ++i)
        for (int f = 0; f < PF_TRACE_FIELDS; ++f) out[i * PF_TRACE_FIELDS + f] = t.rec[(t.count - n + i) % PF_TRACE_LEN][f];
    return n;
}

static int filter_run_checked(const pf_filter_args* A, int64_t t0, int64_t n_steps, int finalize, void* stream,
                              float* kernel_ms, ThetaFold* theta);

extern "C" int pf_filter_run(const pf_filter_args* A, int64_t t0, int64_t n_steps, int finalize, void* stream) {
    return filter_run_checked(A, t0, n_steps, finalize, stream, nullptr, nullptr);
}

extern "C" int pf_filter_observe(const pf_filter_args* A, int64_t t0, int64_t n_steps, int finalize, void* w, const void* ll, void* stats,
                                 void* host_slot, uint64_t seq, void* acc, void* stream) {
    if (!A || !w || !ll || !stats || ((uintptr_t)host_slot & 7) != 0) return PF_EINVAL;
    ThetaFold tf{w, ll, stats, host_slot, seq, acc, 0};
    const int rc = filter_run_checked(A, t0, n_steps, finalize, stream, nullptr, &tf);
    if (rc != PF_OK) return rc;
    if (tf.folded) return PF_OK;
    return pf_theta_step(w, ll, A->B, A->dtype, stats, host_slot, seq, acc, A->status, stream);
}

extern "C" int pf_filter_run_timed(const pf_filter_args* A, int64_t t0, int64_t n_steps, int finalize, void* stream,
                                   float* kernel_ms) {
    if (!kernel_ms) return PF_EINVAL;
    return filter_run_checked(A, t0, n_steps, finalize, stream, kernel_ms, nullptr);
}

struct PfGraph {
    hipGraph_t graph;
    hipGraphExec_t exec;
};

extern "C" int pf_filter_graph_create(const pf_filter_args* A, int64_t t0, int64_t n_steps, int finalize, void* stream,
                                      void** handle) {
    if (!handle) return PF_EINVAL;
    *handle = nullptr;
    (void)stream;
    hipStream_t st = nullptr;
    hipError_t e = hipStreamCreateWithFlags(&st, hipStreamNonBlocking);
    if (e != hipSuccess) return (int)e;
    e = hipStreamBeginCapture(st, hipStreamCaptureModeThreadLocal);
    if (e != hipSuccess) {
        (void)hipStreamDestroy(st);
        return (int)e;
    }
    const int rc = filter_run_checked(A, t0, n_steps, finalize, (void*)st, nullptr, nullptr);
    hipGraph_t graph = nullptr;
    e = hipStreamEndCapture(st, &graph);
    (void)hipStreamDestroy(st);
    if (rc != PF_OK) {
        if (graph) (void)hipGraphDestroy(graph);
        return rc;
    }
    if (e != hipSuccess) return (int)e;
    hipGraphExec_t exec = nullptr;
    e = hipGraphInstantiate(&exec, graph, nullptr, nullptr, 0);
    if (e != hipSuccess) {
        (void)hipGraphDestroy(graph);
        return (int)e;
    }
    PfGraph* g = new PfGraph{graph, exec};
    *handle = g;
    return PF_OK;
}

extern "C" int pf_filter_graph_launch(void* handle, void* stream) {
    if (!handle) return PF_EINVAL;
    const hipError_t e = hipGraphLaunch(((PfGraph*)handle)->exec, (hipStream_t)stream);
    return e == hipSuccess ? PF_OK : (int)e;
}

extern "C" int pf_filter_graph_destroy(void* handle) {
    if (!handle) return PF_OK;
    PfGraph* g = (PfGraph*)handle;
    (void)hipGraphExecDestroy(g->exec);
    (void)hipGraphDestroy(g->graph);
    delete g;
    return PF_OK;
}

static int filter_run_checked(const pf_filter_args* A, int64_t t0, int64_t n_steps, int finalize, void* stream,
                              float* kernel_ms, ThetaFold* theta) {
    if (!A || A->struct_size != sizeof(pf_filter_args)) return PF_EINVAL;
    if (A->hints.route < 0 || A->hints.route > PF_ROUTE_CLUSTER_SPREAD || A->hints.column_max_n < 0 || A->hints.tile_target < 0 ||
        A->hints.cluster_patience < -1 || A->hints.cluster_patience > (1 << 30) || A->hints.cluster_generation < 0)
        return PF_EINVAL;
    int rc = check_model(&A->model, true);
    if (rc) return rc;
    if (bad_shape(A->N, A->B) || t0 < 0 || n_steps < 0) return PF_EINVAL;
    if (A->ring < 0 || A->ring == 1) return PF_EINVAL;
    if (A->hints.prepare_next != 0) {
        if (A->filter != PF_FILTER_APF || finalize || n_steps < 1) return PF_EINVAL;
        if (A->model.hid_kind == PF_HID_USER_AFFINE && (A->proposal != PF_PROP_LGO || !A->user_scale_per_column)) return PF_EINVAL;
    }
    if (!A->x[0] || !A->logw[0] || (A->ring < 3 && (!A->x[1] || !A->logw[1])) || !A->anc || !A->cdf || !A->means || !A->vars ||
        !A->ll_steps || !A->ll_total || !A->ws)
        return PF_EINVAL;
    if (n_steps > 0 && (!A->y || (!A->observed && !A->observed_dev && n_steps > PF_AUTO_FLAGS))) return PF_EINVAL;
    if (A->y_rows != 1 && A->y_rows != A->B) return PF_EINVAL;
    if (A->proposal == PF_PROP_LGO && A->model.obs_kind != PF_OBS_LINEAR) return PF_EUNSUPPORTED;
    if (A->model.hid_kind == PF_HID_USER_AFFINE) {
        if (!A->user_loc || !A->user_scale) return PF_EINVAL;
        if (n_steps > 1 || A->ring >= 3) return PF_EUNSUPPORTED;
    }
    if (A->filter != PF_FILTER_SISR && A->filter != PF_FILTER_APF) return PF_EUNSUPPORTED;
    if (!A->pos) return PF_EINVAL;
    const Geom g = make_geom(A->N, A->B, A->hints.tile_target);
    const WsLayout wl = make_ws(g);
    if (A->ws_bytes < wl.total) return PF_EWORKSPACE;
    hipStream_t st = (hipStream_t)stream;
    if (!column_eligible(A, g, n_steps, finalize) && cluster_eligible(A, g, n_steps, finalize) && wl.clu_bytes != 0) {
        if (A->dtype != PF_F32 && A->dtype != PF_F64) return PF_EINVAL;
        rc = A->dtype == PF_F32 ? pf_run_cluster_f32(A, g, wl, t0, n_steps, st, kernel_ms, theta)
                                : pf_run_cluster_f64(A, g, wl, t0, n_steps, st, kernel_ms, theta);
        if (rc != PF_CLUSTER_INFEASIBLE) return rc;
    }
    if (column_eligible(A, g, n_steps, finalize)) {
        if (A->dtype == PF_F32) return pf_run_column_f32(A, g, wl, t0, n_steps, st, kernel_ms);
        if (A->dtype == PF_F64) return pf_run_column_f64(A, g, wl, t0, n_steps, st, kernel_ms);
        return PF_EINVAL;
    }
    return with_dtype(A->dtype, [&](auto t) {
        return with_d3(A->model.dim, [&](auto d) {
            return with_vec(g.vec, [&](auto v) {
                return with_bool(g.rounds_per_tile > 1, [&](auto multi) {
                    return filter_run_impl<decltype(t), decltype(d)::value, decltype(v)::value, decltype(multi)::value>(A, g, wl, t0, n_steps,
                                                                                                                  finalize, st, kernel_ms);
                });
            });
        });
    });
}
```

### pyfilter_amd/csrc/pf_models.hpp

```cpp
#pragma once
#include "pf_device.hpp"

#define PF_MAXD 3
#define PF_MAXO 3

#include "../../include/pf_amd.h"

namespace pf {

#define PF_LOG_SQRT_2PI 0.91893853320467274178

template <int D> struct ObsDim {
    static constexpr int MAXO = (D == 1) ? 1 : PF_MAXO;
};

template <typename T, int D> struct ColParams {
    static constexpr int MAXO = ObsDim<D>::MAXO;
    T hp[4][D];
    T A[MAXO][D];
    T ob[MAXO];
    T os[MAXO];
    T y[MAXO];
    T yn[MAXO];
    int O;
// ... 137 lines not shown
            ob = cp.ob[0];
            i2s = T(0.5) * ovi;
            ks = pf_log_c(s) + T(PF_LOG_SQRT_2PI);
            i2inc = T(0.5) * pf_rcp_c(inc * inc);
            kt = pf_log_c(inc * pf_abs(g)) + T(PF_LOG_SQRT_2PI);
            cov = pf_rcp_c(hvi + a * ovi * a);
            c_loc = cov * hvi;
            c_y = cov * (a * (ovi * yb));
            kstd = pf_sqrt_c(cov);
            kq = T(0.5) * pf_log_c(cov) + T(PF_LOG_SQRT_2PI);
            const T cvar = s * s + a * (g * g) * a;
            i2c = T(0.5) * pf_rcp_c(cvar);
            kc = T(0.5) * pf_log_c(cvar) + T(PF_LOG_SQRT_2PI);
        }
    }
    __device__ __forceinline__ void prepare_user(const ModelDesc& md, const ColParams<T, D>& cp, T g_user) {
        if constexpr (D == 1) {
            if (md.obs_kind != PF_OBS_LINEAR) return;
            fast = true;
            g = g_user;
            ou_e = T(0);
            finish_fast(md, cp);
        }
    }

    __device__ __forceinline__ void set_obs(const ColParams<T, D>& cp) {
        if constexpr (D == 1) {
            if (!fast) return;
            yb = cp.y[0] - cp.ob[0];
            ybn = cp.yn[0] - cp.ob[0];
            c_y = cov * (a * (ovi * yb));
        }
    }

    __device__ __forceinline__ T loc1(const ModelDesc& md, const ColParams<T, D>& cp, T x) const {
        switch (md.hid_kind) {
            case PF_HID_LINEAR: return cp.hp[0][0] + cp.hp[1][0] * x;
            case PF_HID_SINE_EM: return x + pf_sin(x - cp.hp[0][0]) * (T)md.dt;
            default: return cp.hp[1][0] + (x - cp.hp[1][0]) * ou_e;
        }
    }
    __device__ __forceinline__ T obs_lp_lin(const ColParams<T, D>& cp, const T (&x)[D], bool next) const {
        T lp = -oks;
#pragma unroll
        for (int o = 0; o < MAXO; ++o) {
            if (o < cp.O) {
                T r = (next ? cp.yn[o] : cp.y[o]) - cp.ob[o];
#pragma unroll
                for (int d = 0; d < D; ++d) r -= cp.A[o][d] * x[d];
                lp -= (r * r) * oi2s[o];
            }
        }
        return lp;
    }
    __device__ __forceinline__ T obs_lp(T x, bool next = false) const {
        const T r = (next ? ybn : yb) - a * x;
        return -(r * r) * i2s - ks;
    }
};

enum {
    PK_A0 = 0, PK_A1, PK_A2, PK_A3, PK_G, PK_INC, PK_A, PK_YB, PK_YBN, PK_I2S, PK_KS, PK_CLOC, PK_CY, PK_KSTD, PK_INVG,
    PK_I2INC, PK_KT, PK_KQ, PK_I2C, PK_KC, PK_OB, PK_OVI, PK_COV, PK_USED, PK_N = 24
};
template <typename T> using const_ptr = const __attribute__((address_space(4))) T*;

template <typename T> __device__ __forceinline__ void write_col_pack(const ModelDesc& md, const ColParams<T, 1>& cp,
                                                                     const ColConsts<T, 1>& cc, T* __restrict__ q) {
    T A0 = T(0), A1 = T(0), A2 = T(0), A3 = T(0);
    switch (md.hid_kind) {
        case PF_HID_LINEAR: A0 = cp.hp[0][0]; A1 = cp.hp[1][0]; break;
        case PF_HID_SINE_EM: A2 = (T)md.dt; A3 = cp.hp[0][0]; break;
        default: A0 = cp.hp[1][0]; A3 = cp.hp[1][0]; A1 = cc.ou_e; break;
    }
    q[PK_A0] = A0; q[PK_A1] = A1; q[PK_A2] = A2; q[PK_A3] = A3;
    q[PK_G] = cc.g; q[PK_INC] = cc.inc; q[PK_A] = cc.a; q[PK_YB] = cc.yb; q[PK_YBN] = cc.ybn;
    q[PK_I2S] = cc.i2s; q[PK_KS] = cc.ks; q[PK_CLOC] = cc.c_loc; q[PK_CY] = cc.c_y; q[PK_KSTD] = cc.kstd;
    q[PK_INVG] = cc.inv_g; q[PK_I2INC] = cc.i2inc; q[PK_KT] = cc.kt; q[PK_KQ] = cc.kq; q[PK_I2C] = cc.i2c; q[PK_KC] = cc.kc;
    q[PK_OB] = cc.ob; q[PK_OVI] = cc.ovi; q[PK_COV] = cc.cov;
}

template <typename T> struct FastCol {
    T A0, A1, A2, A3, g, inc, a, yb, ybn, i2s, ks, c_loc, c_y, kstd, inv_g, i2inc, kt, kq, i2c, kc;
    __device__ __forceinline__ void load(const_ptr<T> q, T y_t, T y_next) {
        A0 = q[PK_A0]; A1 = q[PK_A1]; A2 = q[PK_A2]; A3 = q[PK_A3];
        g = q[PK_G]; inc = q[PK_INC]; a = q[PK_A];
        i2s = q[PK_I2S]; ks = q[PK_KS]; c_loc = q[PK_CLOC]; kstd = q[PK_KSTD];
        inv_g = q[PK_INVG]; i2inc = q[PK_I2INC]; kt = q[PK_KT]; kq = q[PK_KQ]; i2c = q[PK_I2C]; kc = q[PK_KC];
        const T ob = q[PK_OB];
        yb = y_t - ob;
        ybn = y_next - ob;
        c_y = q[PK_COV] * (a * (q[PK_OVI] * yb));
    }
    template <int LK = 0> __device__ __forceinline__ T loc(T x) const {
        if constexpr (LK == 1) return A0 + (x - A3) * A1;
        if constexpr (LK == 2) return x + pf_sin_fast(x - A3) * A2;
        if (A2 != T(0)) return x + pf_sin_fast(x - A3) * A2;
        return A0 + (x - A3) * A1;
    }
    __device__ __forceinline__ T obs_lp(T x, bool next = false) const {
        const T r = (next ? ybn : yb) - a * x;
        return -(r * r) * i2s - ks;
    }
    template <int LK = 0> __device__ __forceinline__ T pre_weight(int proposal, T x, bool next = false) const {
        if (proposal == PF_PROP_BOOTSTRAP) return obs_lp(loc<LK>(x), next);
        const T r = (next ? ybn : yb) - a * x;
        return -(r * r) * i2c - kc;
    }
    template <int LK = 0> __device__ __forceinline__ T sample_and_weight_apf(int proposal, T x, T z, T& xn, T& pre) const {
        const T l = loc<LK>(x);
        if (proposal == PF_PROP_BOOTSTRAP) {
            pre = obs_lp(l);
            xn = l + g * (z * inc);
            return obs_lp(xn);
        }
        const T r = yb - a * x;
        pre = -(r * r) * i2c - kc;
        const T km = c_loc * l + c_y;
        xn = km + kstd * z;
        const T eps = (xn - l) * inv_g;
        return obs_lp(xn) + (-(eps * eps) * i2inc - kt) - (-T(0.5) * z * z - kq);
    }
    template <int LK = 0> __device__ __forceinline__ T sample_and_weight(int proposal, T x, T z, T& xn) const {
        const T l = loc<LK>(x);
        if (proposal == PF_PROP_BOOTSTRAP) {
            xn = l + g * (z * inc);
            return obs_lp(xn);
        }
        const T km = c_loc * l + c_y;
        xn = km + kstd * z;
        const T eps = (xn - l) * inv_g;
        return obs_lp(xn) + (-(eps * eps) * i2inc - kt) - (-T(0.5) * z * z - kq);
    }
};

template <typename T> __device__ __forceinline__ T normal_logpdf(T y, T loc, T scale) {
    const T r = y - loc;
    if constexpr (sizeof(T) == 4) {
        const T z = r * pf_rcp_c(scale);
        return T(-0.5) * (z * z) - pf_log_c(scale) - T(PF_LOG_SQRT_2PI);
    } else {
        return -(r * r) / (T(2) * scale * scale) - pf_log(scale) - T(PF_LOG_SQRT_2PI);
    }
}

template <typename T, int D>
__device__ __forceinline__ T obs_logpdf(const ModelDesc& md, const ColParams<T, D>& cp, const T (&x)[D], bool next = false) {
    if (md.obs_kind == PF_OBS_SV) return normal_logpdf(next ? cp.yn[0] : cp.y[0], cp.ob[0], x[0]);
    T lp = T(0);
#pragma unroll
    for (int o = 0; o < ColParams<T, D>::MAXO; ++o) {
        if (o < cp.O) {
            T loc = cp.ob[o];
#pragma unroll
            for (int d = 0; d < D; ++d) loc += cp.A[o][d] * x[d];
            lp += normal_logpdf(next ? cp.yn[o] : cp.y[o], loc, cp.os[o]);
        }
    }
    return lp;
}

template <typename T, int D>
__device__ __forceinline__ T transition_logpdf(const ModelDesc& md, const T (&xn)[D], const T (&loc)[D],
                                               const T (&scale)[D]) {
    const T inc = (T)md.inc_scale;
    T lp = T(0);
    if constexpr (sizeof(T) == 4) {
// ... 250 lines not shown
```

### pyfilter_amd/csrc/pf_step.hip

```cpp
#include "pf_host.hpp"

#define PF_STEP_KERNELS_f32d1_v4 1
#define PF_STEP_KERNELS_f32d1_v1 2
#define PF_STEP_KERNELS_f32dn 3
#define PF_STEP_KERNELS_f64 4
#define PF_STEP_CAT2(a, b) a##b
#define PF_STEP_CAT(a, b) PF_STEP_CAT2(a, b)
#ifndef PF_STEP_KERNELS
#error "pf_step.hip: -DPF_STEP_KERNELS=f32d1_v4|f32d1_v1|f32dn|f64 is required"
#endif
#define PF_STEP_SET PF_STEP_CAT(PF_STEP_KERNELS_, PF_STEP_KERNELS)
#if PF_STEP_SET < 1 || PF_STEP_SET > 4
#error "pf_step.hip: PF_STEP_KERNELS must be one of f32d1_v4, f32d1_v1, f32dn, f64"
#endif
#ifndef PF_STEP_MULTI
#error "pf_step.hip: -DPF_STEP_MULTI=0|1 is required"
#endif
#if PF_STEP_MULTI != 0 && PF_STEP_MULTI != 1
#error "pf_step.hip: PF_STEP_MULTI must be 0 or 1"
#endif

#define PF_BOOK_INLINE_TILES 1
template <typename T, int D, int VEC, bool MULTI>
int filter_run_impl(const pf_filter_args* A, const Geom& g, const WsLayout& wl, int64_t t0, int64_t n_steps, int finalize,
                    hipStream_t st, float* kernel_ms) {
    FusedArgs<T> a = make_fused_args<T>(A, g, wl, t0);

    const dim3 grid_tiles(g.tiles, g.B), block(PF_BLOCK);
    a.book_inline = g.tiles < PF_BOOK_INLINE_TILES ? 1 : 0;
#ifdef PF_DEVTOOLS
    if (const char* bi = getenv("PF_BOOK_INLINE")) a.book_inline = atoi(bi);
#endif
    a.kmap = 0u;
    if (g.B == 1 && g.tiles >= 16 && (g.tiles & (g.tiles - 1)) == 0) {
        unsigned q = 0;
        while ((1 << q) < g.tiles) ++q;
        a.kmap = 7u | ((q - 3u) << 8) | (3u << 16);
    }
    const dim3 grid(g.B, g.tiles + (a.book_inline ? 0 : 1));
    const ObsFlags<T> flags(A, wl, t0, n_steps);
    if (t0 == 0) {
        const size_t words = (wl.off_ctr - wl.off_stat) / sizeof(uint32_t);
        flags.launch_zero((uint32_t*)((char*)A->ws + wl.off_stat), words, flags.derive, n_steps, st);
    }
    const int64_t ring = A->ring >= 3 ? A->ring : 0;
    auto place = [&](int64_t t) {
        if (!ring) return;
        const int64_t rs = t % ring, wsl = (t + 1) % ring, bn = (int64_t)g.B * g.N;
        a.x[t & 1] = (T*)A->x[0] + rs * D * bn;
        a.x[(t + 1) & 1] = (T*)A->x[0] + wsl * D * bn;
        a.logw[t & 1] = (T*)A->logw[0] + rs * bn;
        a.logw[(t + 1) & 1] = (T*)A->logw[0] + wsl * bn;
        a.anc = A->anc + wsl * bn;
        a.anc_prev = A->anc + rs * bn;
    };
    place(t0);
    a.step = (int)t0;
    a.obs_dev = flags.dev;
    if (flags.derive && t0 != 0) flags.launch_derive(n_steps, st);
    a.obs = n_steps > 0 ? flags.obs(t0) : 0;
    a.obs_next = 0;
    const bool resumed = A->hints.resume != 0 && t0 > 0 && A->ring < 3;
    const bool prepare_next = A->hints.prepare_next != 0 && A->filter == PF_FILTER_APF && !finalize && n_steps > 0;
    if (!resumed) hipLaunchKernelGGL((k_fused_reduce<T, D, VEC>), grid_tiles, block, 0, st, a);

    const bool force_search = A->hints.ancestor_search != 0;
    const int mode = (A->resampler == PF_RESAMPLE_MULTINOMIAL)
                         ? 1
                         : ((sizeof(T) == 4 && (g.N > ((int64_t)1 << 22) || force_search)) ? 2 : 0);
    auto spec_of = [&]() -> int {
        if (sizeof(T) != 4 || a.z_tape || a.obs != 1) return 0;
        if (a.md.hid_kind == PF_HID_USER_AFFINE && a.filter == PF_FILTER_APF) return 0;
        if (a.filter == PF_FILTER_APF) return a.obs_next == 1 ? 1 : 0;
        return 2;
    };
    auto launch_step_as = [&](auto prop_c, auto fast_c) {
        constexpr int PROP = decltype(prop_c)::value;
        constexpr bool FAST = decltype(fast_c)::value;
        auto go = [&](auto mode_c, auto spec_c) {
            constexpr int MODE = decltype(mode_c)::value;
            constexpr int SPEC = decltype(spec_c)::value;
            auto launch = [&](auto mk_c) {
                constexpr int MK = decltype(mk_c)::value;
                trace_launch((int)a.step, (int)sizeof(T), D, VEC, MODE, PROP, FAST ? 1 : 0, SPEC, MK, MULTI ? 1 : 0);
                hipLaunchKernelGGL((k_fused_step<T, D, VEC, MODE, PROP, FAST, SPEC, MK, MULTI>), grid, block, 0, st, a);
            };
            if constexpr (!FAST) {
                if (a.md.hid_kind == PF_HID_USER_AFFINE) {
                    if constexpr (SPEC != 1) launch(std::integral_constant<int, 3>{});
                    return;
                }
            }
            if constexpr (sizeof(T) == 4 && !FAST && D == 1) {
                if (a.md.hid_kind == PF_HID_VERHULST_EM && a.md.obs_kind == PF_OBS_SV) return launch(std::integral_constant<int, 1>{});
            }
            if constexpr (sizeof(T) == 4 && !FAST && D == 3) {
                if (a.md.hid_kind == PF_HID_LORENZ63_EM && a.md.obs_kind == PF_OBS_LINEAR)
                    return launch(std::integral_constant<int, 4>{});
            }
            if constexpr (sizeof(T) == 4 && FAST && D == 1) {
                if (a.md.hid_kind == PF_HID_SINE_EM) return launch(std::integral_constant<int, 2>{});
                return launch(std::integral_constant<int, 1>{});
            }
            launch(std::integral_constant<int, 0>{});
        };
        auto with_mode = [&](auto mode_c) {
            if constexpr (sizeof(T) == 4) {
                const int sp = spec_of();
                if (sp == 1) return go(mode_c, std::integral_constant<int, 1>{});
                if (sp == 2) return go(mode_c, std::integral_constant<int, 2>{});
            }
            go(mode_c, std::integral_constant<int, 0>{});
        };
        if (mode == 0) with_mode(std::integral_constant<int, 0>{});
        else if (mode == 1) with_mode(std::integral_constant<int, 1>{});
        else if constexpr (sizeof(T) == 4) go(std::integral_constant<int, 2>{}, std::integral_constant<int, 0>{});
    };
    auto launch_step = [&]() {
        bool fast = false;
        if constexpr (D == 1)
            fast = a.md.obs_kind == PF_OBS_LINEAR && a.md.hid_kind != PF_HID_VERHULST_EM && a.md.hid_kind != PF_HID_USER_AFFINE;
        if (fast) {
            if constexpr (D == 1) {
                if (a.proposal == PF_PROP_BOOTSTRAP) launch_step_as(std::integral_constant<int, PF_PROP_BOOTSTRAP>{}, std::true_type{});
                else launch_step_as(std::integral_constant<int, PF_PROP_LGO>{}, std::true_type{});
            }
        } else if (a.proposal == PF_PROP_BOOTSTRAP) {
            launch_step_as(std::integral_constant<int, PF_PROP_BOOTSTRAP>{}, std::false_type{});
        } else {
            launch_step_as(std::integral_constant<int, PF_PROP_LGO>{}, std::false_type{});
        }
    };
    const KernelTimer timer(kernel_ms, st);
    if (timer.failed) return timer.rc;
    for (int64_t s = 0; s < n_steps; ++s) {
        const int64_t t = t0 + s;
        a.step = (int)t;
        place(t);
        a.obs = flags.obs(t);
        a.obs_next = (s + 1 < n_steps) ? flags.obs(t + 1) : (prepare_next ? 1 : 0);
        a.keep_state = (ring != 0 || s + 1 == n_steps) ? 1 : 0;
#ifdef PF_DEVTOOLS
        if (a.debug_cut != 0) a.keep_state = 1;
        static const bool cut_at_end = getenv("PF_DEBUG_CUT_AT_END") != nullptr;
        const int cut_all = a.debug_cut;
        if (cut_at_end && cut_all > 0 && s != n_steps - 2) a.debug_cut = 0;
#endif
        launch_step();
#ifdef PF_DEVTOOLS
        a.debug_cut = cut_all;
#endif
    }
    timer.stop();
    if (finalize) {
        a.step = (int)(t0 + n_steps);
        a.obs = a.obs_next = 0;
        a.finalize_only = 1;
        hipLaunchKernelGGL((k_fused_book<T, D>), dim3(1, g.B), block, 0, st, a);
    }
    if (const int rc = timer.finish(n_steps)) return rc;
    return launch_status();
}

#define PF_LEAF_AT(T, D, VEC, MULTI) \
    template int filter_run_impl<T, D, VEC, MULTI>(const pf_filter_args*, const Geom&, const WsLayout&, int64_t, int64_t, int, hipStream_t, float*);
#define PF_LEAF(T, D, VEC) PF_LEAF_AT(T, D, VEC, PF_STEP_MULTI != 0)
// ... 12 lines not shown
```

### pyfilter_amd/filters/particle/base.py

```python
import ctypes as C
from typing import Callable, Optional, Union

import torch

from ... import _lib as L
from ... import ops
from ...hints import HINTS, ROUTE_AUTO, ROUTE_CLUSTER, ROUTE_PER_STEP
from ...resampling import multinomial, systematic
from ...timeseries import AffineEulerMaruyama, StateSpaceModel, TimeseriesState
from ...timeseries.models import pack_params
from ..base import BaseFilter
from ..result import FilterResult
from ..schedule import expand
from .forecast import Forecast, kernel_applies, kernel_forecast, normalized_weights, torch_forecast
from .proposals import Bootstrap, LinearGaussianObservations, Proposal
from .proposals.base import KernelContext
from .state import ParticleFilterCorrection, ParticleFilterPrediction

_DEFAULT_SEED = 2024
_GOLD = 0x9E3779B97F4A7C15
_M64 = 0xFFFFFFFFFFFFFFFF


class ParticleFilter(BaseFilter[ParticleFilterCorrection, ParticleFilterPrediction]):
    _FILTER_KIND = None

    def __init__(
        self,
        model,
        particles: int,
        resampling: Callable[[torch.Tensor], torch.Tensor] = systematic,
        proposal: Union[str, Proposal] = None,
        ess_threshold=0.9,
        seed: Optional[int] = None,
        **kwargs,
    ):
        super().__init__(model, **kwargs)
        self._base_particles = torch.Size([particles])
        self._resample_threshold = ess_threshold * particles
        self._resampler = resampling
        self._proposal: Proposal = proposal if proposal is not None else Bootstrap()
        self._seed = _DEFAULT_SEED if seed is None else int(seed)
        self._ctx: Optional[KernelContext] = None
        self._z_tape = None
        self._u_tape = None
        self._z0 = None
        self._fused_plans = {}
        self._single_plans = {}
        self._single_last = None
        self._move_by_move = False
        self._draws = 0
        self._copies = 0
        self._forecasts = 0
        self._obs_cache = None
        self.cluster_fallbacks = 0
        self._time_kernels, self.kernel_ms = False, None
        self._last_run = self._keep_planes = None
        self._u_gen = self._percol_cache = self._ffbs_u = None

    @property
    def particles(self) -> torch.Size:
        return torch.Size([*self._base_particles, *self.batch_shape])

    @property
    def proposal(self) -> Proposal:
        return self._proposal

    def increase_particles(self, factor: int):
        self._base_particles = torch.Size([int(factor * self._base_particles[0])])
        self._resample_threshold *= factor
        self._ctx = None

    def initialize_model(self, context):
        super().initialize_model(context)
        self._proposal.set_model(self._model)
        self._ctx = None

    def set_tape(self, z: Optional[torch.Tensor] = None, u: Optional[torch.Tensor] = None, z0: Optional[torch.Tensor] = None):
        self._z_tape, self._u_tape, self._z0 = z, u, z0
        self._ctx = None

    @property
    def _batched(self) -> bool:
        return len(self.batch_shape) > 0

    @property
    def _has_event(self) -> bool:
        return self._model.hidden.n_dim > 0

    def _device_dtype(self):
# ... 221 lines not shown
        apf = self._FILTER_KIND == L.FILTER_APF
        x_out, lw_out = torch.empty_like(x_in), torch.empty_like(lw_in)
        if apf:
            anc = torch.empty((b, n), device=device, dtype=torch.int32)
        else:
            own = state._anc32 is not None
            anc = state.ancestors32().clone() if own else state.ancestors32().reshape(b, n).contiguous()
        mean_new, var_new, ll_new, stats_ptr = plan.zeroed_stats(batched)
        es = plan.elem_size
        a = plan.args
        verified = watched and HINTS.kernel_route() == ROUTE_CLUSTER and HINTS.cluster_takes(n, b, rs_kind == L.RESAMPLE_SYSTEMATIC)
        stream = L.stream_ptr()
        hk = (HINTS.key(), verified, stream)
        if plan.hints_key != hk or a.hints.prepare_next:
            plan.write_hints(hk, ROUTE_AUTO if (HINTS.kernel_route() == ROUTE_CLUSTER and not verified) else None)
        if verified:
            ll_into = None
        a.model.params = ctx.params.data_ptr()
        planes = None
        if kind.is_user:
            loc, scale, a.user_dt = self._user_mean_scale(self._model.hidden, ts_in)
            full = ts_in.value.shape
            percol = self._scale_per_column(scale, full, dtype)
            planes = (ops.to_soa(loc.to(dtype).expand(full), batched, has_event).contiguous(),
                      percol if percol is not None else ops.to_soa(scale.to(dtype).expand(full), batched, has_event).contiguous())
            a.user_loc, a.user_scale = planes[0].data_ptr(), planes[1].data_ptr()
            a.user_scale_per_column = 0 if percol is None else 1
        m = 0
        per_step_route = (not verified) and (HINTS.route == ROUTE_PER_STEP or (a.hints.route == ROUTE_AUTO and n > (HINTS.column_max_n or 2048)))
        chain = plan.chain
        if (per_step_route and chain is not None and chain[1] is x_in and chain[2] is lw_in and chain[3] == x_in._version
                and chain[4] == lw_in._version and chain[5] == hk):
            m = chain[0] + 1
        plan.chain = None
        resume = 1 if (m > 0 and not apf) else 0
        if a.hints.resume != resume:
            a.hints.resume = resume
        a.y, a.y_rows = y_dev.data_ptr() - m * rows * o * es, rows
        a.observed, a.observed_dev, a.step_counter = None, None, None
        a.seed = self._next_draw_seed()
        a.x[m & 1], a.x[(m + 1) & 1] = x_in.data_ptr(), x_out.data_ptr()
        a.logw[m & 1], a.logw[(m + 1) & 1] = lw_in.data_ptr(), lw_out.data_ptr()
        a.anc = anc.data_ptr()
        db = d * b * es
        a.means, a.vars = stats_ptr - m * db, stats_ptr + 2 * db - m * db
        a.ll_steps = stats_ptr + 4 * db - m * b * es
        ll_added = (ll_into is not None and ll_into.device == device and ll_into.dtype == dtype and ll_into.numel() == b
                    and ll_into.is_contiguous())
        a.ll_total = ll_into.data_ptr() if ll_added else stats_ptr + 4 * db + b * es
        z_tape = u_tape = None
        if ctx.z_tape is not None:
            z_tape = ctx.z_tape[t_start:t_start + 1].contiguous()
            assert z_tape.shape[0] == 1, "z tape shorter than the number of steps"
        if ctx.u_tape is not None:
            u_tape = ctx.u_tape[t_start:t_start + 1].contiguous()
        a.z_tape = None if z_tape is None else z_tape.data_ptr() - m * d * b * n * es
        a.u_tape = None if u_tape is None else u_tape.data_ptr() - m * b * es
        a.hints.cluster_generation = plan.next_generation()
        L.check(plan.run(plan.args_ref, m, 1, 1, stream), "pf_filter_run")
        if per_step_route:
            plan.chain = (m, x_out, lw_out, x_out._version, lw_out._version, hk)
        self._last_run = dict(plan=plan, z=z_tape, u=u_tape, ws=plan.ws, seed_eff=a.seed, piece=m,
                              keep=(x_in, lw_in, y_dev, ctx.params, planes))
        watch = None
        if verified:
            pool_row = plan._pool[0][plan._pool_next - 1]

            def restore():
                if not apf:
                    anc.copy_(state.ancestors32().reshape(b, n))
                pool_row[4 * d + 1].zero_()

            watch = (plan.status, lambda: self._reissue_per_step(plan, restore, 0, 1))

        x_view, w_view = plan.state_views(x_out, lw_out, batched, has_event)
        new = ParticleFilterCorrection(TimeseriesState(t_start + 1, x_view, self._model.hidden.event_shape), w_view, ll_new, None,
                                       _moments=(mean_new, var_new), _anc32=(anc, batched))
        new._soa = (x_view, w_view, x_out, lw_out)
        return new, ll_added, watch

    def batch_filter(self, y, bar=True, init_state=None) -> FilterResult:
        return self._batch_filter(y, init_state, bar=bar)[0]

    def _batch_filter(self, y, init_state=None, *, bar=False, defer_status=False, per_step=False):
        assert self._model is not None, "Model has not been initialized!"
        device, _ = self._device_dtype()
        if (not self._fused_capable(device) or not isinstance(y, torch.Tensor)
                or not HINTS.fused_batch
                or (self._kernel_kind().is_user and FilterResult.states_kept(self.record_states) != 1)):
            return super().batch_filter(y, bar=bar, init_state=init_state), None
        if self._single_launch_run(y):
            return self._batch_filter_lean(y, init_state, defer_status, per_step)
        return self._batch_filter_fused(y, init_state), None

    def _single_launch_run(self, y) -> bool:
        return (y.shape[0] > 0 and FilterResult.states_kept(self.record_states) == 1 and not self._time_kernels
                and not self._move_by_move and not self._kernel_kind().is_user and int(self._model.observe_every_step) == 1
                and (HINTS.direct or (HINTS.route != ROUTE_PER_STEP and self._base_particles[0] <= (HINTS.column_max_n or 2048))
                     or HINTS.cluster_takes(self._base_particles[0], self.batch_shape[0] if self._batched else 1,
                                            self._resampler_kind() == L.RESAMPLE_SYSTEMATIC))
                and self._ctx_tapes_none())

    def _batch_filter_lean(self, y: torch.Tensor, init_state, defer_status: bool, per_step: bool):
        state = init_state if init_state is not None else self.initialize()
        result = FilterResult(state, self.record_states, self.record_moments, _defer_moments=True)
        blk, _, _ = self._filter_block_lean(y, state, None, None, host_u=True, defer_status=defer_status, per_step=per_step)
        result._extend_fused(blk.filter_means, blk.filter_variance, blk.loglikelihood, blk.latest_state)
        self._last_run["rows"] = (blk.filter_means, blk.filter_variance)
        return result, ((blk.status, blk.plan) if blk.status is not None else None)

    def _observed_flags(self, y: torch.Tensor, y_dev: torch.Tensor) -> torch.Tensor:
        cached = self._obs_cache
        if cached is not None and cached[0] is y and cached[1] == y._version:
            return cached[2]
        flags = ops.observed_flags(y_dev).cpu()
        self._obs_cache = (y, y._version, flags)
        return flags

    def filter_block(self, y: torch.Tensor, state: ParticleFilterCorrection, observed: Optional[torch.Tensor] = None,
                     replay=None, per_step: bool = False, defer_status: bool = False):
        x = state.timeseries_state.value
        if (not self._fused_capable(x.device) or int(self._model.observe_every_step) != 1 or self._record_intermediary
                or self._kernel_kind().is_user):
            return None
        if (FilterResult.states_kept(self.record_states) == 1 and not self._time_kernels
                and not self._move_by_move and self._ctx_tapes_none()):
            return self._filter_block_lean(y, state, observed, replay, per_step=per_step, defer_status=defer_status)
        res = self._batch_filter_fused(y, state._restarted(), observed=observed, replay=replay)
        res.status = None
        run = self._last_run
        res.block_rows = (run["rows"][0][1:].clone(), run["rows"][1][1:].clone())
        ll = run["ll_steps"]
        u = run["u"]
        return res, (ll if self._batched else ll[:, 0]), (run["seed_eff"], None if u is None else u.clone())

    @staticmethod
    def _user_mean_scale(hidden, ts):
        if type(hidden) is AffineEulerMaruyama:
            fg = hidden.drift_scale(ts)
            if fg is not None:
                return fg
        loc, scale = hidden.mean_scale(ts)
        return loc, scale, 0.0

    def _scale_per_column(self, scale: torch.Tensor, full, dtype) -> Optional[torch.Tensor]:
        if scale.dim() != len(full) or scale.shape != full or scale.stride(0) != 0:
            return None
        key = (scale.data_ptr(), scale._version, tuple(scale.stride()), dtype)
        cached = self._percol_cache
        if cached is not None and cached[0] == key:
            return cached[1]
        out = self._scale_rows(scale, dtype)
        self._percol_cache = (key, out, scale)
        return out

    def _scale_rows(self, scale: torch.Tensor, dtype) -> torch.Tensor:
        row = scale[0].to(dtype)
        if not self._batched:
            row = row.unsqueeze(0)
        row = row.reshape(row.shape[0], -1)
        return row.t().contiguous()

    def _ctx_tapes_none(self) -> bool:
        ctx = self._ensure_context()
        return ctx.z_tape is None and ctx.u_tape is None

    def online_run(self, result: FilterResult):
        return _OnlineRun(self, result) if _OnlineRun.applies(self, result) else None

    def _single_plan(self, kind, n, b, d, o, rows, dtype, device):
        key = (n, b, d, o, rows, dtype, device, self._FILTER_KIND, self._proposal._KERNEL_PROPOSAL,
               self._resampler_kind(), float(self._resample_threshold))
        plan = self._single_plans.get(key)
        if plan is None:
            plan = self._single_plans[key] = _SingleStepPlan(self, kind, n, b, d, o, rows, dtype, device)
        return plan

    def _cluster_gave_up(self, plan):
        plan.status.zero_()
        self.cluster_fallbacks += 1
        if self.cluster_fallbacks == 1:
            import warnings

            warnings.warn("pyfilter_amd: a column-cluster launch gave up waiting for its sibling workgroups (the device was held "
                          "by other work); the piece is re-issued on the per-step route - same draws, same results")

    def _reissue_per_step(self, plan, restore, t0: int, n_steps: int):
        self._cluster_gave_up(plan)
        restore()
        plan.write_hints(None, ROUTE_PER_STEP)
        L.check(plan.run(plan.args_ref, t0, n_steps, 1, L.stream_ptr()), "pf_filter_run")

    def _filter_block_lean(self, y: torch.Tensor, state: ParticleFilterCorrection, observed, replay, host_u: bool = False,
                           per_step: bool = False, defer_status: bool = False):
        ctx = self._ctx
        kind = ctx.kind
        ts_in = state.timeseries_state
        x_in = ops.to_soa(ts_in.value, self._batched, self._has_event)
        lw_in = ops.to_cols(state.weights)
        device, dtype = x_in.device, x_in.dtype
        d, b, n = x_in.shape
        o = kind.obs_dim
        steps = y.shape[0]
        y_dev = y.to(device=device, dtype=dtype).reshape(steps, -1, o)
        if not y_dev.is_contiguous():
            y_dev = y_dev.contiguous()
        rows = y_dev.shape[1]
        if rows not in (1, b):
            raise L.PfAmdError(f"observations of shape {tuple(y.shape)} do not broadcast against batch {b}")
        flags = (observed if observed is not None else self._observed_flags(y, y_dev)).contiguous()
        plan = self._single_plan(kind, n, b, d, o, rows, dtype, device)
        plan.chain = None
        if plan.xl is None:
            plan.xl = torch.empty((d + 1, b, n), device=device, dtype=dtype)
        t_start = int(ts_in.time_index)

        xl_out = torch.empty((d + 1, b, n), device=device, dtype=dtype)
        anc = torch.empty((b, n), device=device, dtype=torch.int32)
        rows_buf = torch.empty((2, steps + 1, b, d), device=device, dtype=dtype)
        ll = torch.zeros((steps + 1, b), device=device, dtype=dtype)
        first = xl_out if steps % 2 == 0 else plan.xl
        other = plan.xl if steps % 2 == 0 else xl_out
        xl_in = getattr(state, "_xl", None)
        packed = (xl_in is not None and xl_in.shape == first.shape and xl_in.dtype == dtype and xl_in.data_ptr() == x_in.data_ptr()
                  and xl_in[d].data_ptr() == lw_in.data_ptr())

        def load_state():
            if packed:
                first.copy_(xl_in)
            else:
                first[:d].copy_(x_in)
                first[d].copy_(lw_in)
            if self._FILTER_KIND != L.FILTER_APF:
                anc.copy_(state.ancestors32().reshape(b, n))

        load_state()
        a = plan.args
        plan.write_hints(None, ROUTE_PER_STEP if per_step else None)
        a.model.params = ctx.params.data_ptr()
        a.y, a.y_rows = y_dev.data_ptr(), rows
        a.observed, a.observed_dev = flags.data_ptr(), None
        seed_eff = self._next_draw_seed() if replay is None else replay[0]
        a.seed, a.step_counter = seed_eff, None
        u_tape = replay[1][:steps].contiguous() if (replay is not None and replay[1] is not None) else None
        if host_u and u_tape is None and self._resampler_kind() == L.RESAMPLE_SYSTEMATIC:
            if plan.u_gen is None:
                plan.u_gen = torch.Generator(device=device)
            plan.u_gen.manual_seed(seed_eff & 0x7FFFFFFFFFFFFFFF)
            u_tape = torch.empty((steps, b), device=device, dtype=dtype).uniform_(generator=plan.u_gen)
        a.z_tape, a.u_tape = None, L.ptr(u_tape)
        a.x[0], a.x[1] = first.data_ptr(), other.data_ptr()
        a.logw[0], a.logw[1] = first[d].data_ptr(), other[d].data_ptr()
        a.anc = anc.data_ptr()
        a.means, a.vars = rows_buf[0].data_ptr(), rows_buf[1].data_ptr()
        a.ll_steps, a.ll_total = ll.data_ptr(), ll[steps].data_ptr()
        a.hints.cluster_generation = plan.next_generation()
        L.check(plan.run(plan.args_ref, 0, steps, 1, L.stream_ptr()), "pf_filter_run")
        watched = (not per_step) and HINTS.cluster_takes(n, b, self._resampler_kind() == L.RESAMPLE_SYSTEMATIC)
        if watched and not defer_status and int(plan.status.item()) != 0:
            self._reissue_per_step(plan, lambda: (load_state(), ll.zero_()), 0, steps)
        self._last_run = dict(plan=plan, z=None, u=u_tape, ws=plan.ws, seed_eff=seed_eff, ll_steps=ll[:steps],
                              keep=(x_in, lw_in, y_dev, flags, ctx.params))

        md = (lambda t: t) if self._batched else (lambda t: t[:, 0])
        means, variances = md(rows_buf[0]), md(rows_buf[1])
        ll_steps = ll[:steps] if self._batched else ll[:steps, 0]
        last = ParticleFilterCorrection(
            TimeseriesState(t_start + steps, ops.from_soa(xl_out[:d], self._batched, self._has_event), self._model.hidden.event_shape),
            ops.from_cols(xl_out[d], self._batched), ll_steps[steps - 1], None,
            _moments=(means[steps], variances[steps]), _anc32=(anc, self._batched),
        )
        last._xl = xl_out
        res = _BlockResult(means, variances, ll[steps] if self._batched else ll[steps, 0], last)
        res.status = plan.status if (watched and defer_status) else None
        res.plan = plan
        return res, ll_steps, (seed_eff, None)

    def _batch_filter_fused(self, y: torch.Tensor, init_state=None, observed=None, replay=None) -> FilterResult:
        state = init_state if init_state is not None else self.initialize()
        ctx = self._ensure_context()
        kind = ctx.kind
        x0 = state.timeseries_state.value
        device, dtype = x0.device, x0.dtype
        n = self._base_particles[0]
        b = self.batch_shape[0] if self._batched else 1
        d, o = kind.dim, kind.obs_dim

        result = FilterResult(state, self.record_states, self.record_moments, _defer_moments=True)
        t_obs = y.shape[0]
        if t_obs == 0:
            result._moments.append(state.get_mean(), state.get_variance(), self._batched)
            return result

        t_start = int(state.timeseries_state.time_index)
        sched = expand(t_start, t_obs, int(self._model.observe_every_step))
        steps = sched.moves
        y_dev = y.to(device=device, dtype=dtype).reshape(t_obs, -1, o)
        if y_dev.shape[1] not in (1, b):
            raise L.PfAmdError(f"observations of shape {tuple(y.shape)} do not broadcast against batch {b}")
        rows = y_dev.shape[1]
        informative = observed if observed is not None else self._observed_flags(y, y_dev)
        if steps == t_obs:
            y_steps, observed_host = y_dev, informative
        else:
            at = torch.tensor(sched.rows)
            observed_host = torch.zeros(steps, dtype=torch.uint8)
            observed_host[at] = informative
            y_steps = torch.full((steps, rows, o), float("nan"), device=device, dtype=dtype)
            y_steps[at.to(device)] = y_dev

        keep_states = FilterResult.states_kept(self.record_states)
        reported = list(range(1, steps + 1)) if (steps == t_obs or self._record_intermediary) else [r + 1 for r in sched.rows]
        if keep_states == 1:
            ring, wanted = 0, reported[-1:]
        else:
            wanted = reported if keep_states is None else reported[-keep_states:]
            ring = max(3, steps - wanted[0] + 1)
        taped = ctx.z_tape is not None or ctx.u_tape is not None
        use_graph = ((not taped) and not ring and replay is None and not self._time_kernels
                     and HINTS.graph and not kind.is_user and not self._move_by_move)
        key = (n, b, d, o, steps, rows, dtype, device, self._FILTER_KIND, self._proposal._KERNEL_PROPOSAL,
               self._resampler_kind(), self._seed, float(self._resample_threshold), observed_host.numpy().tobytes(), HINTS.key())
        user_graph = (kind.is_user and bool(getattr(self._model.hidden, "graph_callable", False)) and (not taped) and not ring
                      and replay is None and not self._time_kernels and HINTS.graph
                      and not isinstance(self._move_by_move, (list, tuple)))
        plan = self._fused_plans.get(key) if (use_graph or user_graph) else None
        if plan is None:
            plan = _FusedPlan(self, kind, n, b, d, o, steps, rows, dtype, device, observed_host, ring=ring)
            if use_graph or user_graph:
                if len(self._fused_plans) >= 4:
                    self._fused_plans.pop(next(iter(self._fused_plans))).destroy()
                self._fused_plans[key] = plan

        def load_state():
            plan.x[0].copy_(ops.to_soa(x0, self._batched, self._has_event))
            plan.logw[0].copy_(ops.to_cols(state.weights))
            (plan.anc_hist[0] if ring else plan.anc).copy_(state.ancestors32().reshape(b, n))
            plan.ll_total.zero_()

        plan.params.copy_(ctx.params)
        load_state()
        plan.y.copy_(y_steps)
        seed_eff = self._next_draw_seed() if replay is None else replay[0]
        word = (seed_eff - self._seed) & _M64
        plan.epoch.fill_(word - (1 << 64) if word >= (1 << 63) else word)
        a = plan.args
        plan.write_hints(None)
        z_tape = u_tape = None
        if ctx.z_tape is not None:
            z_tape = ctx.z_tape[t_start:t_start + steps].contiguous()
            assert z_tape.shape[0] == steps, "z tape shorter than the number of steps"
        if ctx.u_tape is not None:
            u_tape = ctx.u_tape[t_start:t_start + steps].contiguous()
        elif replay is not None and replay[1] is not None:
            u_tape = replay[1][:steps].contiguous()
        elif self._resampler_kind() == L.RESAMPLE_SYSTEMATIC:
            plan.u_gen.manual_seed(seed_eff & 0x7FFFFFFFFFFFFFFF)
            plan.u.uniform_(generator=plan.u_gen)
            u_tape = plan.u
        a.z_tape, a.u_tape = L.ptr(z_tape), L.ptr(u_tape)

        lib = L.load()
        if kind.is_user or self._move_by_move:
            hidden, full = self._model.hidden, x0.shape
            es_u = hidden.event_shape
            chained = kind.is_user and (HINTS.route == ROUTE_PER_STEP or n > (HINTS.column_max_n or 2048))
            keep = []
            apf_lgo = self._FILTER_KIND == L.FILTER_APF and self._proposal._KERNEL_PROPOSAL == L.PROP_LGO
            prepared_with = None
            if not kind.is_user and isinstance(self._move_by_move, (list, tuple)):
                t_piece = 0
                for n_piece, fin in self._move_by_move:
                    n_piece = steps - t_piece if n_piece is None else n_piece
                    L.check(lib.pf_filter_run(C.byref(a), t_piece, n_piece, fin, L.stream_ptr()), "pf_filter_run")
                    t_piece += n_piece
                assert t_piece == steps, "the pieces do not cover the run"
            def issue_moves():
                nonlocal keep, prepared_with
                for s_ in range(steps if (kind.is_user or not isinstance(self._move_by_move, (list, tuple))) else 0):
                    if not kind.is_user:
                        L.check(lib.pf_filter_run(C.byref(a), s_, 1, 1, L.stream_ptr()), "pf_filter_run")
                        continue
                    ts = TimeseriesState(t_start + s_, ops.from_soa(plan.x[s_ & 1], self._batched, self._has_event), es_u)
                    loc, scale, a.user_dt = self._user_mean_scale(hidden, ts)
                    v = ops.to_soa(loc.to(dtype).expand(full), self._batched, self._has_event)
                    loc_p = v if v.is_contiguous() else plan.user_loc.copy_(v)
                    percol = self._scale_per_column(scale, full, dtype)
                    if percol is not None:
                        scale_p = percol
                    else:
                        v = ops.to_soa(scale.to(dtype).expand(full), self._batched, self._has_event)
                        scale_p = v if v.is_contiguous() else plan.user_scale.copy_(v)
                    keep = [loc_p, scale_p]
                    a.user_loc, a.user_scale = loc_p.data_ptr(), scale_p.data_ptr()
                    a.user_scale_per_column = 0 if percol is None else 1
                    last_move = s_ == steps - 1
                    a.hints.resume = 1 if (chained and s_ > 0 and (self._FILTER_KIND == L.FILTER_SISR or
                                                                   (prepared_with is not None and percol is prepared_with))) else 0
                    prepare = bool(chained and apf_lgo and percol is not None and not last_move and observed_host[s_ + 1])
                    a.hints.prepare_next = 1 if prepare else 0
                    prepared_with = percol if prepare else None
                    L.check(lib.pf_filter_run(C.byref(a), s_, 1, 1 if (last_move or not chained) else 0, L.stream_ptr()), "pf_filter_run")

            captured = False
            if user_graph and plan.runs >= 1 and not plan.user_graph_failed:
                sig = (id(ctx),) + tuple(p.data_ptr() for p in hidden.parameters if isinstance(p, torch.Tensor))
                if plan.user_graph is None or plan.user_graph_sig != sig:
                    graph = torch.cuda.CUDAGraph()
                    self._percol_cache = None
                    try:
                        with torch.cuda.graph(graph, capture_error_mode="thread_local"):
                            issue_moves()
                        plan.user_graph, plan.user_graph_sig, plan.user_graph_keep = graph, sig, (list(keep), self._percol_cache)
                        self._percol_cache = None
                    except Exception as e:
                        import warnings

                        plan.user_graph, plan.user_graph_failed = None, True
                        self._percol_cache = None
                        warnings.warn(f"graph_callable: capturing the callable failed ({type(e).__name__}: {e}); the run is issued eagerly")
                        torch.cuda.synchronize()
                if plan.user_graph is not None:
                    plan.user_graph.replay()
                    captured = True
            if not captured:
                issue_moves()
            if kind.is_user:
                a.user_loc, a.user_scale = plan.user_loc.data_ptr(), plan.user_scale.data_ptr()
                a.user_scale_per_column, a.hints.resume, a.hints.prepare_next = 0, 0, 0
                self._keep_planes = keep
# ... 406 lines not shown
```

### pyfilter_amd/hints.py

```python

ROUTE_AUTO, ROUTE_PER_STEP, ROUTE_COLUMN_GENERIC, ROUTE_CLUSTER, ROUTE_CLUSTER_ALWAYS, ROUTE_CLUSTER_SPREAD = 0, 1, 2, 3, 4, 5


class RunHints:
    __slots__ = ("route", "column_max_n", "tile_target", "ancestor_search", "fused_step", "fused_batch", "graph", "direct",
                 "theta_kernels", "cluster", "cluster_patience", "nested_kernel")

    def __init__(self):
        self.reset()

    def reset(self):
        self.route = ROUTE_AUTO
        self.cluster = True
        self.cluster_patience = 0
        self.column_max_n = 0
        self.tile_target = 0
        self.ancestor_search = 0
        self.fused_step = True
        self.fused_batch = True
        self.graph = True
        self.theta_kernels = True
        self.nested_kernel = True
        self.direct = False

    def key(self):
        return (self.kernel_route(), self.column_max_n, self.tile_target, self.ancestor_search, self.cluster_patience)

    def kernel_route(self):
        return ROUTE_CLUSTER if (self.route == ROUTE_AUTO and self.cluster) else self.route

    def cluster_takes(self, n, b, resampler_systematic=True):
        route = self.kernel_route()
        if route not in (ROUTE_CLUSTER, ROUTE_CLUSTER_ALWAYS, ROUTE_CLUSTER_SPREAD) or not resampler_systematic:
            return False
        if n <= max(2048, self.column_max_n or 2048) or n > 16384 or n % 4:
            return False
        members = ((n + 1023) // 1024) * b
        return members <= 2048 if route == ROUTE_CLUSTER else members <= 8192

    def fill(self, args):
        h = args.hints
        h.route, h.column_max_n, h.tile_target, h.ancestor_search = self.kernel_route(), self.column_max_n, self.tile_target, self.ancestor_search
        h.cluster_patience = self.cluster_patience
        h.cluster_generation = 0
        h.resume = h.prepare_next = 0

    def apply_mapping(self, m):
        on = lambda k: str(m.get(k, "0")) not in ("", "0")
        self.route = ROUTE_PER_STEP if on("PF_NO_COLUMN") else (ROUTE_COLUMN_GENERIC if on("PF_COLUMN_GENERIC") else
                                                                (ROUTE_CLUSTER_ALWAYS if on("PF_CLUSTER") else ROUTE_AUTO))
        self.cluster = not on("PF_NO_CLUSTER")
        self.column_max_n = int(m.get("PF_COLUMN_MAX_N", 0) or 0)
        self.tile_target = int(m.get("PF_TARGET_WGS", 0) or 0)
        self.ancestor_search = 1 if on("PF_FORCE_SEARCH") else 0
        self.fused_step, self.fused_batch, self.graph = not on("PF_NO_FUSED_STEP"), not on("PF_NO_FUSED_BATCH"), not on("PF_NO_GRAPH")
        self.direct = on("PF_DIRECT")
        self.theta_kernels = not on("PF_NO_THETA_KERNELS")
        self.nested_kernel = not on("PF_NO_NESTED_KERNEL")
        self.cluster_patience = int(m.get("PF_CLUSTER_PATIENCE", 0) or 0)
        return self


HINTS = RunHints()
```

### pyfilter_amd/ops.py

```python
import ctypes as C
import os
from typing import Optional, Tuple

import torch

from . import _lib as L


def to_cols(w: torch.Tensor) -> torch.Tensor:
    if w.dim() == 1:
        return w.contiguous().unsqueeze(0)
    if w.dim() != 2:
        raise L.PfAmdError("weights must be (N,) or (N, B): nested batches are not supported (filters/base.py:116-119)")
    return w.t().contiguous()


def from_cols(c: torch.Tensor, batched: bool) -> torch.Tensor:
    return c.t() if batched else c[0]


def to_soa(x: torch.Tensor, batched: bool, has_event: bool) -> torch.Tensor:
    if not has_event:
        x = x.unsqueeze(-1)
    if not batched:
# ... 263 lines not shown
                                      L.stream_ptr()),
        "pf_sample_and_weight",
    )
    return x_out, w_out


def nested_sample_and_weight_soa(kind, params, m: int, x: torch.Tensor, y: torch.Tensor, z: Optional[torch.Tensor],
                                 v: Optional[torch.Tensor], seed: int, step: int, want_pick: bool = False):
    L.require_gpu(x, y, z, v, params)
    d, b, n = x.shape
    x_out = torch.empty_like(x)
    w_out = torch.empty((b, n), dtype=x.dtype, device=x.device)
    pick = torch.empty((b, n), dtype=torch.int32, device=x.device) if want_pick else None
    yy, rows = _y_rows(y.to(x.dtype), b, kind.obs_dim)
    if z is not None:
        assert tuple(z.shape) == (m, d, b, n) and z.is_contiguous() and z.dtype == x.dtype
    if v is not None:
        assert tuple(v.shape) == (b, n) and v.is_contiguous() and v.dtype == x.dtype
    assert x.is_contiguous()
    mod = make_model_struct(kind, params)
    L.check(
        L.load().pf_nested_sample_and_weight(C.byref(mod), int(m), L.ptr(x), L.ptr(yy), rows, L.ptr(z), L.ptr(v), seed, step,
                                             L.ptr(x_out), L.ptr(w_out), L.ptr(pick), n, b, L.dtype_code(x.dtype), L.stream_ptr()),
        "pf_nested_sample_and_weight",
    )
    return x_out, w_out, pick


def forecast_soa(kind, params, steps: int, x: torch.Tensor, W: Optional[torch.Tensor], z: Optional[torch.Tensor] = None,
                 e: Optional[torch.Tensor] = None, seed: int = 0, paths: bool = False):
    L.require_gpu(x, W, z, e, params)
    d, b, n = x.shape
    o, steps = int(kind.obs_dim), int(steps)
    dt, dev = x.dtype, x.device
    assert x.is_contiguous()
    if W is not None:
        assert tuple(W.shape) == (b, n) and W.is_contiguous() and W.dtype == dt
    if z is not None:
        assert tuple(z.shape) == (steps, d, b, n) and z.is_contiguous() and z.dtype == dt
    if e is not None:
        assert tuple(e.shape) == (steps, o, b, n) and e.is_contiguous() and e.dtype == dt
    rows = max(steps, 0)
    moments = [torch.empty((rows, b, k), dtype=dt, device=dev) for k in (d, d, o, o)]
    x_path = torch.empty((rows, d, b, n), dtype=dt, device=dev) if paths else None
    y_path = torch.empty((rows, o, b, n), dtype=dt, device=dev) if paths else None
    nbytes = C.c_size_t(0)
    if steps >= 1:
        L.check(L.load().pf_forecast_workspace_bytes(n, b, steps, C.byref(nbytes)), "pf_forecast_workspace_bytes")
    ws = torch.empty(max(nbytes.value, 8), dtype=torch.uint8, device=dev)
    mod = make_model_struct(kind, params)
    L.check(
        L.load().pf_forecast(C.byref(mod), steps, L.ptr(x), L.ptr(W), L.ptr(z), L.ptr(e), int(seed) & 0xFFFFFFFFFFFFFFFF,
                             *[m.data_ptr() for m in moments], L.ptr(x_path), L.ptr(y_path), ws.data_ptr(), ws.numel(), n, b,
                             L.dtype_code(dt), L.stream_ptr()),
        "pf_forecast",
    )
    return (*moments, x_path, y_path)


def initial_sample_soa(m0, s0, n: int, b: int, d: int, dtype, device, seed: int, z: Optional[torch.Tensor] = None):
    x = torch.empty((d, b, n), dtype=dtype, device=device)
    L.require_gpu(x, z)
    am = (C.c_double * d)(*[float(v) for v in m0])
    asd = (C.c_double * d)(*[float(v) for v in s0])
    L.check(
        L.load().pf_initial_sample(am, asd, L.ptr(z), seed, L.ptr(x), n, b, d, L.dtype_code(dtype), L.stream_ptr()),
        "pf_initial_sample",
    )
    return x


def initial_sample_cols(m0: torch.Tensor, s0: torch.Tensor, n: int, b: int, d: int, seed: int, z: Optional[torch.Tensor] = None):
    assert tuple(m0.shape) == (b, d) and tuple(s0.shape) == (b, d) and m0.dtype == s0.dtype and m0.device == s0.device
    x = torch.empty((d, b, n), dtype=m0.dtype, device=m0.device)
    L.require_gpu(x, z, m0, s0)
    (mb, md), (sb, sd) = m0.stride(), s0.stride()
    L.check(L.load().pf_initial_sample_cols(m0.data_ptr(), mb, md, s0.data_ptr(), sb, sd, L.ptr(z), seed, x.data_ptr(), n, b, d,
                                            L.dtype_code(x.dtype), L.stream_ptr()), "pf_initial_sample_cols")
    return x


SYNC_CHECKS = False

TRACE_FIELDS = ("step", "tbytes", "D", "VEC", "MODE", "PROP", "FAST", "SPEC", "MK", "MULTI")


def debug_draw_normals(seed: int, steps: int, n: int, b: int, d: int, dtype, device, step0: int = 0) -> torch.Tensor:
    out = torch.empty((steps, d, b, n), dtype=dtype, device=device)
    L.require_gpu(out)
    L.check(L.load().pf_debug_draw_normals(seed & 0xFFFFFFFFFFFFFFFF, step0, steps, out.data_ptr(), n, b, d,
                                           L.dtype_code(dtype), L.stream_ptr()), "pf_debug_draw_normals")
    return out


TRACE_LEN = 2048


def debug_launch_trace(last: int = 64):
    buf = (C.c_int32 * (len(TRACE_FIELDS) * last))()
    n = L.load().pf_debug_launch_trace(buf, last)
    if n < 0:
        L.check(n, "pf_debug_launch_trace")
    k = len(TRACE_FIELDS)
    return [dict(zip(TRACE_FIELDS, buf[i * k:(i + 1) * k])) for i in range(n)]


def observed_flags(y: torch.Tensor) -> torch.Tensor:
    L.require_gpu(y)
    y = y.contiguous()
    steps = y.shape[0]
    out = torch.empty(steps, dtype=torch.uint8, device=y.device)
    if steps:
        L.check(L.load().pf_observed_flags(y.data_ptr(), steps, y.numel() // steps, L.dtype_code(y.dtype), out.data_ptr(),
                                           L.stream_ptr()), "pf_observed_flags")
    return out


def theta_ess(log_w: torch.Tensor) -> torch.Tensor:
    L.require_gpu(log_w)
    log_w = log_w.contiguous()
    b = log_w.shape[-1]
    rows = log_w.numel() // b
    out = torch.empty(log_w.shape[:-1] + (2,), dtype=log_w.dtype, device=log_w.device)
    L.check(L.load().pf_theta_ess(log_w.data_ptr(), rows, b, L.dtype_code(log_w.dtype), out.data_ptr(), L.stream_ptr()),
            "pf_theta_ess")
    return out


def theta_path(w0: torch.Tensor, ll: torch.Tensor, rows: Optional["HostRows"] = None, status: Optional[torch.Tensor] = None):
    L.require_gpu(w0, ll)
    n, b = ll.shape
    assert w0.shape == (b,) and w0.dtype == ll.dtype and w0.is_contiguous() and ll.is_contiguous()
    assert rows is None or rows.n >= n
    w_path = torch.empty_like(ll)
    stats = torch.empty((n, 2), dtype=ll.dtype, device=ll.device)
    rp, seq = (None, 0) if rows is None else (rows.ptr, rows.seq + 1)
    L.check(L.load().pf_theta_path(w0.data_ptr(), ll.data_ptr(), n, b, L.dtype_code(ll.dtype), w_path.data_ptr(), stats.data_ptr(),
                                   rp, seq, L.ptr(status) if rows is not None else None, L.stream_ptr()), "pf_theta_path")
    if rows is not None:
        rows.seq = seq
    return w_path, stats


def _free_host(ptr: int):
    try:
        L.load().pf_host_free(ptr)
    except Exception:
        pass


class HostSlot:

    SPINS = 1 << 22

    def __init__(self):
        import weakref

        p = C.c_void_p()
        L.check(L.load().pf_host_alloc(64, C.byref(p)), "pf_host_alloc")
        self.ptr = p.value
        self._vals = (C.c_double * 2).from_address(self.ptr)
        self._seq = C.c_uint64.from_address(self.ptr + 16)
        self._status = C.c_uint64.from_address(self.ptr + 24)
        self.seq = 0
        fin = weakref.finalize(self, _free_host, self.ptr)
        fin.atexit = False

    def __deepcopy__(self, memo):
        return HostSlot()

    def wait(self):
        want, cell = self.seq, self._seq
        for _ in range(self.SPINS):
            if cell.value == want:
                break
        else:
            torch.cuda.current_stream().synchronize()
            if cell.value != want:
                raise L.PfAmdError("pf_theta_step: the device's write to the host slot never became visible")
        self.status = int(self._status.value)
        return self._vals[0], self._vals[1]


class HostRows:

# ... 166 lines not shown
```

Measured before the change: 78.82 billion particle-steps/s.

## Add specialized one-column fused-step leaf with precomputed scalar header

Adds a specialized k_fused_step instantiation for the single-filter f32 D=1 APF+LGO systematic case. The host precomputes a compact per-step header of resolved pointers, and the kernel preloads scalars into SGPRs, so per-step address arithmetic, kernarg indirection and branching on batch index are skipped. The generic path stays reachable through a new PER_STEP_GENERIC route, and the launch trace gains a field. This adds a host-side header build per step and extra code-path complexity, and the narrow eligibility conditions may leave the new path unused.

After: 89.18 billion particle-steps/s (median of 6 runs). 1.13x the previous value.

```diff
diff --git a/include/pf_amd.h b/include/pf_amd.h
--- a/include/pf_amd.h
+++ b/include/pf_amd.h
@@ -161,6 +161,7 @@
 #define PF_ROUTE_CLUSTER 3
 #define PF_ROUTE_CLUSTER_ALWAYS 4
 #define PF_ROUTE_CLUSTER_SPREAD 5
+#define PF_ROUTE_PER_STEP_GENERIC 6
 typedef struct pf_run_hints {
     int32_t route;
     int32_t column_max_n;
@@ -234,6 +235,7 @@
                           int dtype, void* stream);
 
 int pf_debug_launch_trace(int32_t* out, int max_records);
+int pf_debug_launch_trace_fields(int32_t* out, int max_records, int fields);
 
 #ifdef __cplusplus
 }
diff --git a/pyfilter_amd/_lib.py b/pyfilter_amd/_lib.py
--- a/pyfilter_amd/_lib.py
+++ b/pyfilter_amd/_lib.py
@@ -23,7 +23,7 @@
     "pf_version", "pf_abi_version", "pf_error_string", "pf_workspace_bytes", "pf_normalize", "pf_systematic", "pf_systematic_cdf_free", "pf_systematic_logw",
     "pf_multinomial", "pf_gather", "pf_loglik", "pf_moments", "pf_pre_weight", "pf_sample_and_weight",
     "pf_initial_sample", "pf_filter_run", "pf_filter_run_timed", "pf_filter_graph_create", "pf_filter_graph_launch",
-    "pf_filter_graph_destroy", "pf_columns_gather", "pf_columns_exchange", "pf_debug_draw_normals", "pf_debug_launch_trace",
+    "pf_filter_graph_destroy", "pf_columns_gather", "pf_columns_exchange", "pf_debug_draw_normals", "pf_debug_launch_trace", "pf_debug_launch_trace_fields",
     "pf_smooth_fixed_lag", "pf_smooth_ffbs", "pf_observed_flags", "pf_theta_ess", "pf_theta_fit", "pf_theta_propose",
     "pf_theta_accept", "pf_theta_path", "pf_theta_resample", "pf_initial_sample_cols", "pf_theta_step", "pf_host_alloc",
     "pf_host_free", "pf_filter_observe", "pf_jitter_fit", "pf_jitter_apply", "pf_nested_sample_and_weight",
@@ -148,6 +148,7 @@
                                     C.POINTER(vp), vp]
     lib.pf_debug_draw_normals.argtypes = [u64, u32, i64, vp, i64, i64, i64, i32, vp]
     lib.pf_debug_launch_trace.argtypes = [C.POINTER(C.c_int32), i32]
+    lib.pf_debug_launch_trace_fields.argtypes = [C.POINTER(C.c_int32), i32, i32]
     for name in EXPORTS:
         fn = getattr(lib, name)
         if name not in ("pf_version", "pf_error_string"):
diff --git a/pyfilter_amd/csrc/pf_fused.hpp b/pyfilter_amd/csrc/pf_fused.hpp
--- a/pyfilter_amd/csrc/pf_fused.hpp
+++ b/pyfilter_amd/csrc/pf_fused.hpp
@@ -93,6 +93,48 @@
     int keep_state;
 };
 
+template <typename T> struct OneColHeader {
+    const double* pm2;
+    const double* ps2;
+    double* part_out;
+    const T* l_in;
+    T* l_out;
+    const T* x_in;
+    T* x_out;
+    const uint64_t* seed_dev;
+    uint64_t seed;
+    const T* cpack;
+    const T* y_t;
+    const T* piv_mean;
+    const double* piv0;
+    const T* u_t;
+    int32_t* poison_cur;
+    int32_t* poison_next;
+    int N, tiles;
+    unsigned kmap;
+    int step;
+    T rcN;
+    int y_rows;
+};
+template <typename T, bool ONECOL> struct StepHeader {};
+template <typename T> struct StepHeader<T, true> {
+    OneColHeader<T> h;
+    uint64_t seed;
+    T u;
+    T y_t, y_n;
+    T piv;
+    T rec[PK_N];
+};
+template <typename T> struct OneColLaunch {
+    OneColHeader<T> h;
+    FusedArgs<T> a;
+};
+template <typename T> __device__ __forceinline__ const FusedArgs<T>& fused_args_of(const FusedArgs<T>& a) { return a; }
+template <typename T> __device__ __forceinline__ const FusedArgs<T>& fused_args_of(const OneColLaunch<T>& l) { return l.a; }
+template <typename T, bool ONECOL> struct StepKernArgs { using type = FusedArgs<T>; };
+template <typename T> struct StepKernArgs<T, true> { using type = OneColLaunch<T>; };
+template <typename V> __device__ __forceinline__ void pin_scalar(const V& v) { asm volatile("" ::"s"(v)); }
+
 template <typename T, int D>
 __device__ __forceinline__ void load_col_params(const FusedArgs<T>& a, int b, int step, bool with_y, ColParams<T, D>& cp,
                                                 int late = 0) {
@@ -779,10 +821,11 @@
     bool resample;
     bool have_z0;
 };
-template <typename T, int D, int VEC, int MODE, int SPEC, bool EARLY_Z, bool MULTI>
-__device__ __forceinline__ StepPlan<T> step_prologue(const FusedArgs<T>& a, const StepShared<T, D, VEC>& sh, T (&z0)[VEC][D]) {
+template <typename T, int D, int VEC, int MODE, int SPEC, bool EARLY_Z, bool MULTI, bool ONECOL = false>
+__device__ __forceinline__ StepPlan<T> step_prologue(const FusedArgs<T>& a, const StepShared<T, D, VEC>& sh, T (&z0)[VEC][D],
+                                                     const StepHeader<T, ONECOL>& hx = StepHeader<T, ONECOL>{}) {
     const Geom& g = a.g;
-    const int b = PF_STEP_B, k = a.tile_of_row(PF_STEP_K);
+    const int b = ONECOL ? 0 : PF_STEP_B, k = a.tile_of_row(PF_STEP_K);
     const int step = a.step;
     const bool obs = SPEC ? true : a.is_obs();
     const bool apf = SPEC ? (SPEC == 1) : (a.filter == PF_FILTER_APF);
@@ -795,7 +838,9 @@
     if (apf && !obs) return pl;
     constexpr bool multinomial = MODE == 1;
     const uint64_t seed = a.seed + (a.seed_dev ? *a.seed_dev : 0ull);
-    const T u_taped = (!multinomial && a.u_tape) ? a.u_tape[(int64_t)step * g.B + b] : T(0);
+    T u_taped;
+    if constexpr (ONECOL) u_taped = hx.u;
+    else u_taped = (!multinomial && a.u_tape) ? a.u_tape[(int64_t)step * g.B + b] : T(0);
     const int64_t stride = (int64_t)g.B * g.tiles;
     const int64_t cb = (int64_t)b * g.tiles;
     double* const redm_d = sh.red + 2 * PF_NWAVES;
@@ -820,7 +865,9 @@
         q1 = two ? 0.0 : part[PQ_Q1 * stride + cb];
     }
     const bool few_tiles = SHORT && !one_tile && g.tiles <= PF_WAVE && a.debug_cut != 79;
-    if (!one_tile && !few_tiles) {
+    if constexpr (ONECOL) {
+        load_col_partials<false, 0>(hx.h.pm2, (int64_t)(hx.h.ps2 - hx.h.pm2), 0, g.tiles, 0, 1, 0, p2);
+    } else if (!one_tile && !few_tiles) {
         if (two) load_col_partials<false, 0>(a.part_r(), stride, cb, g.tiles, PQ_M2, PQ_S2, 0, p2);
         else load_col_partials<true, 0>(a.part_r(), stride, cb, g.tiles, PQ_M1, PQ_S1, 0, p1);
     }
@@ -934,9 +981,9 @@
     PF_STAMP(a, 2);
     return pl;
 }
-template <typename T, int D, int VEC, int MODE, int PROP, bool FAST, int SPEC, int MK, bool RS, bool MULTI>
+template <typename T, int D, int VEC, int MODE, int PROP, bool FAST, int SPEC, int MK, bool RS, bool MULTI, bool ONECOL = false>
 __device__ __forceinline__ void step_body(const FusedArgs<T>& a, const StepShared<T, D, VEC>& sh, const StepPlan<T>& pl,
-                                          const T (&z0)[VEC][D]) {
+                                          const T (&z0)[VEC][D], const StepHeader<T, ONECOL>& hx = StepHeader<T, ONECOL>{}) {
     const int proposal = (PROP >= 0) ? PROP : a.proposal;
     ModelDesc md = a.md;
     if constexpr (!FAST && MK == 1) { md.hid_kind = PF_HID_VERHULST_EM; md.obs_kind = PF_OBS_SV; md.obs_dim = 1; }
@@ -956,7 +1003,7 @@
     T* const redm = sh.redm;
     int* hd = reinterpret_cast<int*>(win);
     const Geom& g = a.g;
-    const int b = PF_STEP_B, k = a.tile_of_row(PF_STEP_K);
+    const int b = ONECOL ? 0 : PF_STEP_B, k = a.tile_of_row(PF_STEP_K);
     const int tid = threadIdx.x;
     const int step = a.step;
     const int slot = step & 1;
@@ -986,8 +1033,15 @@
     }
     const T ub = pl.ub;
 
-    const T* x_in = a.x[slot];
-    const T* lw_in = a.logw[slot] + (int64_t)b * g.N;
+    const T* x_in;
+    const T* lw_in;
+    if constexpr (ONECOL) {
+        x_in = hx.h.x_in;
+        lw_in = nullptr;
+    } else {
+        x_in = a.x[slot];
+        lw_in = a.logw[slot] + (int64_t)b * g.N;
+    }
 #ifdef PF_DEVTOOLS
     T* lw_out = a.logw[slot ^ 1] + (int64_t)b * g.N;
     int32_t* anc_col = a.anc + (int64_t)b * g.N;
@@ -1026,7 +1080,9 @@
     constexpr bool single = !MULTI;
     const bool use_lds = g.rounds_per_tile * PF_NWAVES <= PF_LDS_CHUNKS;
     double* const ct_tile = a.ctab_w(step + 1, b) + 2 * (int64_t)k * g.rounds_per_tile * PF_NWAVES;
-    T* const l_next = ((step & 1) ? a.cdf : a.pos) + (int64_t)b * g.N;
+    T* l_next;
+    if constexpr (ONECOL) l_next = hx.h.l_out;
+    else l_next = ((step & 1) ? a.cdf : a.pos) + (int64_t)b * g.N;
     int rk = 0;
     for (int r = 0; r < g.rounds_per_tile; ++r) {
         const int64_t r0 = base + (int64_t)r * g.round_elems;
@@ -1211,12 +1267,16 @@
         }
 #endif
 
-        int late;
-        asm volatile("v_readfirstlane_b32 %0, %1\n\ts_and_b32 %0, %0, 0" : "=s"(late) : "v"(idx[0]) : "scc");
+        int late = 0;
+        if constexpr (!ONECOL) asm volatile("v_readfirstlane_b32 %0, %1\n\ts_and_b32 %0, %0, 0" : "=s"(late) : "v"(idx[0]) : "scc");
         using KArgs = const __attribute__((address_space(4))) FusedArgs<T>;
         KArgs* la = (KArgs*)((const_ptr<char>)__builtin_amdgcn_kernarg_segment_ptr() + late);
-        T* const x_out = la->x[slot ^ 1];
-        if constexpr (FAST) {
+        T* x_out;
+        if constexpr (ONECOL) x_out = hx.h.x_out;
+        else x_out = la->x[slot ^ 1];
+        if constexpr (ONECOL) {
+            fc.load(&hx.rec[0], hx.y_t, hx.y_n);
+        } else if constexpr (FAST) {
             const_ptr<T> yq = (const_ptr<T>)(uintptr_t)a.y + late;
             const int yc = a.y_rows == 1 ? 0 : b;
             const T y_t = obs ? yq[(int64_t)step * a.y_rows + yc] : T(0);
@@ -1298,7 +1358,8 @@
                 if (j & 1) __builtin_amdgcn_sched_barrier(0);
             }
             PF_STAMP(a, 12);
-            const bool keep = la->keep_state != 0;
+            bool keep = false;
+            if constexpr (!ONECOL) keep = la->keep_state != 0;
             const bool st_anc = keep || !apf;
             const bool st_lw = keep || !(apf && obs && pre_next);
 #pragma unroll
@@ -1329,9 +1390,13 @@
             }
 #endif
             T piv[D];
-#pragma unroll
-            for (int d = 0; d < D; ++d)
-                piv[d] = (step - 1 >= a.t0) ? la->means[((int64_t)(step - 1) * g.B + b) * D + d] : (T)la->piv0[(int64_t)b * PF_MAXD + d];
+            if constexpr (ONECOL) {
+                piv[0] = hx.piv;
+            } else {
+#pragma unroll
+                for (int d = 0; d < D; ++d)
+                    piv[d] = (step - 1 >= a.t0) ? la->means[((int64_t)(step - 1) * g.B + b) * D + d] : (T)la->piv0[(int64_t)b * PF_MAXD + d];
+            }
             if constexpr (MULTI) {
 #pragma unroll
                 for (int j = 0; j < VEC; ++j) {
@@ -1356,7 +1421,11 @@
         }
         if (windowed && r + 1 < g.rounds_per_tile) __syncthreads();
     }
-    if (poison) atomicOr(&a.poison[(step & 3) * g.B + b], 1);
+    if constexpr (ONECOL) {
+        if (poison) atomicOr(hx.h.poison_cur, 1);
+    } else {
+        if (poison) atomicOr(&a.poison[(step & 3) * g.B + b], 1);
+    }
     if (PF_CUT(a, 3)) return;
     PF_STAMP(a, 14);
     T M1, M2, F1, F2;
@@ -1365,7 +1434,16 @@
     const int64_t i0s = base + tid * VEC;
     const bool on_s = i0s < g.N;
     double e[VEC], local = 0.0, incl = 0.0;
-    acc.template finish<MODE == 1>(a.part_w(step + 1), b, k, g.B, g.tiles, single && pre_next, red, redm, &a.poison[((step + 1) & 3) * g.B + b], M1, M2, F1, F2,
+    double* part_next;
+    int32_t* poison_next;
+    if constexpr (ONECOL) {
+        part_next = hx.h.part_out;
+        poison_next = hx.h.poison_next;
+    } else {
+        part_next = a.part_w(step + 1);
+        poison_next = &a.poison[((step + 1) & 3) * g.B + b];
+    }
+    acc.template finish<MODE == 1>(part_next, b, k, g.B, g.tiles, single && pre_next, red, redm, poison_next, M1, M2, F1, F2,
         [&](T f1, T f2) {
             if (!tile_scan) return;
             const T f = pre_next ? f2 : f1;
@@ -1428,8 +1506,9 @@
 #endif
 }
 
-template <typename T, int D, int VEC, int MODE, int PROP, bool FAST, int SPEC, int MK, bool MULTI>
-__global__ __launch_bounds__(PF_BLOCK, (StepWaves<T, D, MODE, PROP, FAST, SPEC, MULTI>::value)) void k_fused_step(FusedArgs<T> a) {
+template <typename T, int D, int VEC, int MODE, int PROP, bool FAST, int SPEC, int MK, bool MULTI, bool ONECOL = false>
+__global__ __launch_bounds__(PF_BLOCK, (StepWaves<T, D, MODE, PROP, FAST, SPEC, MULTI>::value)) void k_fused_step(
+    typename StepKernArgs<T, ONECOL>::type ka) {
     using SH = StepShared<T, D, VEC>;
     __shared__ __attribute__((aligned(32))) T win[SH::WIN];
     __shared__ __attribute__((aligned(32))) T xwin[SH::XWIN ? D * SH::WIN : VEC];
@@ -1442,6 +1521,63 @@
     __shared__ int sh_plan[2];
     __shared__ double crec[MULTI ? 2 * PF_LDS_CHUNKS : 2];
     __shared__ double redb[PF_NWAVES];
+    if constexpr (ONECOL) {
+        static_assert(sizeof(T) == 4 && D == 1 && VEC == 4 && MODE == 0 && FAST && SPEC == 1 && !MULTI, "the one-column leaf's shape");
+        static_assert(sizeof(OneColHeader<T>) <= 192, "the header is fetched with three 64-byte scalar loads");
+        StepHeader<T, true> hx;
+        hx.h = ka.h;
+        OneColHeader<T>& h = hx.h;
+        pin_scalar(h.pm2); pin_scalar(h.ps2); pin_scalar(h.part_out); pin_scalar(h.l_in); pin_scalar(h.l_out); pin_scalar(h.x_in);
+        pin_scalar(h.x_out); pin_scalar(h.seed_dev); pin_scalar(h.seed); pin_scalar(h.cpack); pin_scalar(h.y_t); pin_scalar(h.piv_mean);
+        pin_scalar(h.piv0); pin_scalar(h.u_t); pin_scalar(h.poison_cur); pin_scalar(h.poison_next); pin_scalar(h.N); pin_scalar(h.tiles);
+        pin_scalar(h.kmap); pin_scalar(h.step); pin_scalar(h.rcN); pin_scalar(h.y_rows);
+        if (PF_STEP_K == (unsigned)h.tiles) {
+            column_bookkeeping<T, D>(ka.a, 0, red, redb);
+            return;
+        }
+        auto word = [](auto* p) { return (const_ptr<std::remove_cv_t<std::remove_pointer_t<decltype(p)>>>)(uintptr_t)p; };
+        const uint64_t epoch = *word(h.seed_dev ? h.seed_dev : (const uint64_t*)h.piv0);
+        const T u = *word(h.u_t ? h.u_t : h.cpack);
+        const T piv_m = *word(h.piv_mean ? h.piv_mean : h.cpack);
+        const double piv_r = *word(h.piv0);
+        hx.y_t = *word(h.y_t);
+        hx.y_n = word(h.y_t)[h.y_rows];
+#pragma unroll
+        for (int q = 0; q < PK_N; ++q) hx.rec[q] = word(h.cpack)[q];
+        {
+            const T(&c)[PK_N] = hx.rec;
+            asm volatile("" ::"s"(epoch), "s"(u), "s"(piv_m), "s"(piv_r), "s"(hx.y_t), "s"(hx.y_n), "s"(c[PK_A0]), "s"(c[PK_A1]),
+                         "s"(c[PK_A2]), "s"(c[PK_A3]), "s"(c[PK_G]), "s"(c[PK_INC]), "s"(c[PK_A]), "s"(c[PK_I2S]), "s"(c[PK_KS]),
+                         "s"(c[PK_CLOC]), "s"(c[PK_KSTD]), "s"(c[PK_INVG]), "s"(c[PK_I2INC]), "s"(c[PK_KT]), "s"(c[PK_KQ]),
+                         "s"(c[PK_I2C]), "s"(c[PK_KC]), "s"(c[PK_OB]), "s"(c[PK_OVI]), "s"(c[PK_COV]));
+        }
+        hx.seed = h.seed + (h.seed_dev ? epoch : 0ull);
+        hx.u = h.u_t ? u : T(0);
+        hx.piv = h.piv_mean ? piv_m : (T)piv_r;
+        FusedArgs<T> v{};
+        v.filter = PF_FILTER_APF;
+        v.g.N = (int64_t)(unsigned)h.N;
+        v.g.B = 1;
+        v.g.vec = VEC;
+        v.g.round_elems = v.g.tile_elems = PF_BLOCK * VEC;
+        v.g.rounds_per_tile = 1;
+        v.g.tiles = h.tiles;
+        v.rcN = h.rcN;
+        v.seed = hx.seed;
+        v.cdf = v.pos = const_cast<T*>(h.l_in);
+        v.u_tape = h.u_t;
+        v.step = h.step;
+        v.obs = v.obs_next = 1;
+        v.kmap = h.kmap;
+        const SH sh{win, xwin, &sh_j0, sh_cl, sh_wm, red, reds, redm, ptl, ftl, sh_plan, crec};
+        T z0[VEC][D];
+#pragma unroll
+        for (int j = 0; j < VEC; ++j) z0[j][0] = T(0);
+        const StepPlan<T> pl = step_prologue<T, D, VEC, MODE, SPEC, true, MULTI, true>(v, sh, z0, hx);
+        step_body<T, D, VEC, MODE, PROP, FAST, SPEC, MK, true, MULTI, true>(v, sh, pl, z0, hx);
+        return;
+    }
+    const FusedArgs<T>& a = fused_args_of(ka);
     if (!a.book_inline && PF_STEP_K == (unsigned)a.g.tiles) {
         column_bookkeeping<T, D>(a, PF_STEP_B, red, redb);
         return;
diff --git a/pyfilter_amd/csrc/pf_host.hpp b/pyfilter_amd/csrc/pf_host.hpp
--- a/pyfilter_amd/csrc/pf_host.hpp
+++ b/pyfilter_amd/csrc/pf_host.hpp
@@ -231,16 +231,17 @@
 }
 
 #define PF_TRACE_LEN 2048
-#define PF_TRACE_FIELDS 10
+#define PF_TRACE_FIELDS 11
 struct LaunchTrace {
     int32_t rec[PF_TRACE_LEN][PF_TRACE_FIELDS];
     uint64_t count;
 };
 LaunchTrace& launch_trace();
-static inline void trace_launch(int step, int tbytes, int d, int vec, int mode, int prop, int fast, int spec, int mk, int multi) {
+static inline void trace_launch(int step, int tbytes, int d, int vec, int mode, int prop, int fast, int spec, int mk, int multi, int leaf = 0) {
     LaunchTrace& t = launch_trace();
     int32_t* r = t.rec[t.count % PF_TRACE_LEN];
     r[0] = step; r[1] = tbytes; r[2] = d; r[3] = vec; r[4] = mode; r[5] = prop; r[6] = fast; r[7] = spec; r[8] = mk; r[9] = multi;
+    r[10] = leaf;
     ++t.count;
 }
 
@@ -299,6 +300,36 @@
 }
 
 template <typename T>
+static OneColHeader<T> make_onecol_header(const FusedArgs<T>& a) {
+    OneColHeader<T> h;
+    const int s = a.step;
+    const int64_t stride = (int64_t)a.g.tiles;
+    h.pm2 = a.part + (int64_t)(s & 1) * a.part_stride + PQ_M2 * stride;
+    h.ps2 = a.part + (int64_t)(s & 1) * a.part_stride + PQ_S2 * stride;
+    h.part_out = a.part + (int64_t)((s + 1) & 1) * a.part_stride;
+    h.l_in = (s & 1) ? a.pos : a.cdf;
+    h.l_out = (s & 1) ? a.cdf : a.pos;
+    h.x_in = a.x[s & 1];
+    h.x_out = a.x[(s & 1) ^ 1];
+    h.seed_dev = a.seed_dev;
+    h.seed = a.seed;
+    h.cpack = a.cpack;
+    h.y_t = a.y + (int64_t)s * a.y_rows;
+    h.piv_mean = (s - 1 >= a.t0) ? a.means + (s - 1) : nullptr;
+    h.piv0 = a.piv0;
+    h.u_t = a.u_tape ? a.u_tape + s : nullptr;
+    h.poison_cur = a.poison + (s & 3);
+    h.poison_next = a.poison + ((s + 1) & 3);
+    h.N = (int)a.g.N;
+    h.tiles = a.g.tiles;
+    h.kmap = a.kmap;
+    h.step = s;
+    h.rcN = a.rcN;
+    h.y_rows = a.y_rows;
+    return h;
+}
+
+template <typename T>
 struct ObsFlags {
     const uint8_t* host;
     const uint8_t* dev;
@@ -418,7 +449,7 @@
 #define PF_COLUMN_MAX_N 2048
 static inline bool column_eligible(const pf_filter_args* A, const Geom& g, int64_t n_steps, int finalize) {
     if (!finalize || n_steps < 1 || A->ring >= 3) return false;
-    if (A->hints.route == PF_ROUTE_PER_STEP) return false;
+    if (A->hints.route == PF_ROUTE_PER_STEP || A->hints.route == PF_ROUTE_PER_STEP_GENERIC) return false;
     const int64_t max_n = A->hints.column_max_n > 0 ? A->hints.column_max_n : PF_COLUMN_MAX_N;
     if (A->N > max_n || column_threads(A->N, PF_COLUMN_VEC) > 1024) return false;
     return column_lds_bytes(A->N, A->model.dim, A->dtype == PF_F64 ? 8 : 4, PF_COLUMN_VEC) <= 64 * 1024;
diff --git a/pyfilter_amd/csrc/pf_kernels.hip b/pyfilter_amd/csrc/pf_kernels.hip
--- a/pyfilter_amd/csrc/pf_kernels.hip
+++ b/pyfilter_amd/csrc/pf_kernels.hip
@@ -1801,15 +1801,16 @@
     static thread_local LaunchTrace t = {};
     return t;
 }
-extern "C" int pf_debug_launch_trace(int32_t* out, int max_records) {
-    if (!out || max_records < 0) return PF_EINVAL;
+extern "C" int pf_debug_launch_trace_fields(int32_t* out, int max_records, int fields) {
+    if (!out || max_records < 0 || fields < 1 || fields > PF_TRACE_FIELDS) return PF_EINVAL;
     const LaunchTrace& t = launch_trace();
     const uint64_t have = t.count < PF_TRACE_LEN ? t.count : PF_TRACE_LEN;
     const int n = (uint64_t)max_records < have ? max_records : (int)have;
     for (int i = 0; i < n; ++i)
-        for (int f = 0; f < PF_TRACE_FIELDS; ++f) out[i * PF_TRACE_FIELDS + f] = t.rec[(t.count - n + i) % PF_TRACE_LEN][f];
+        for (int f = 0; f < fields; ++f) out[i * fields + f] = t.rec[(t.count - n + i) % PF_TRACE_LEN][f];
     return n;
 }
+extern "C" int pf_debug_launch_trace(int32_t* out, int max_records) { return pf_debug_launch_trace_fields(out, max_records, 10); }
 
 static int filter_run_checked(const pf_filter_args* A, int64_t t0, int64_t n_steps, int finalize, void* stream,
                               float* kernel_ms, ThetaFold* theta);
@@ -1890,7 +1891,7 @@
 static int filter_run_checked(const pf_filter_args* A, int64_t t0, int64_t n_steps, int finalize, void* stream,
                               float* kernel_ms, ThetaFold* theta) {
     if (!A || A->struct_size != sizeof(pf_filter_args)) return PF_EINVAL;
-    if (A->hints.route < 0 || A->hints.route > PF_ROUTE_CLUSTER_SPREAD || A->hints.column_max_n < 0 || A->hints.tile_target < 0 ||
+    if (A->hints.route < 0 || A->hints.route > PF_ROUTE_PER_STEP_GENERIC || A->hints.column_max_n < 0 || A->hints.tile_target < 0 ||
         A->hints.cluster_patience < -1 || A->hints.cluster_patience > (1 << 30) || A->hints.cluster_generation < 0)
         return PF_EINVAL;
     int rc = check_model(&A->model, true);
diff --git a/pyfilter_amd/csrc/pf_models.hpp b/pyfilter_amd/csrc/pf_models.hpp
--- a/pyfilter_amd/csrc/pf_models.hpp
+++ b/pyfilter_amd/csrc/pf_models.hpp
@@ -243,7 +243,7 @@
 
 template <typename T> struct FastCol {
     T A0, A1, A2, A3, g, inc, a, yb, ybn, i2s, ks, c_loc, c_y, kstd, inv_g, i2inc, kt, kq, i2c, kc;
-    __device__ __forceinline__ void load(const_ptr<T> q, T y_t, T y_next) {
+    template <typename Q> __device__ __forceinline__ void load(Q q, T y_t, T y_next) {
         A0 = q[PK_A0]; A1 = q[PK_A1]; A2 = q[PK_A2]; A3 = q[PK_A3];
         g = q[PK_G]; inc = q[PK_INC]; a = q[PK_A];
         i2s = q[PK_I2S]; ks = q[PK_KS]; c_loc = q[PK_CLOC]; kstd = q[PK_KSTD];
diff --git a/pyfilter_amd/csrc/pf_step.hip b/pyfilter_amd/csrc/pf_step.hip
--- a/pyfilter_amd/csrc/pf_step.hip
+++ b/pyfilter_amd/csrc/pf_step.hip
@@ -82,6 +82,15 @@
             constexpr int SPEC = decltype(spec_c)::value;
             auto launch = [&](auto mk_c) {
                 constexpr int MK = decltype(mk_c)::value;
+                if constexpr (sizeof(T) == 4 && D == 1 && VEC == 4 && !MULTI && MODE == 0 && FAST && SPEC == 1 && (MK == 1 || MK == 2)) {
+                    if (A->hints.route != PF_ROUTE_PER_STEP_GENERIC && g.B == 1 && a.kmap != 0u && g.N <= ((int64_t)1 << 22) &&
+                        !a.z_tape && !ring && a.obs == 1 && a.obs_next == 1 && a.keep_state == 0 && !a.book_inline && a.debug_cut == 0) {
+                        trace_launch((int)a.step, (int)sizeof(T), D, VEC, MODE, PROP, 1, SPEC, MK, 0, 1);
+                        hipLaunchKernelGGL((k_fused_step<T, D, VEC, MODE, PROP, FAST, SPEC, MK, MULTI, true>), grid, block, 0, st,
+                                           OneColLaunch<T>{make_onecol_header<T>(a), a});
+                        return;
+                    }
+                }
                 trace_launch((int)a.step, (int)sizeof(T), D, VEC, MODE, PROP, FAST ? 1 : 0, SPEC, MK, MULTI ? 1 : 0);
                 hipLaunchKernelGGL((k_fused_step<T, D, VEC, MODE, PROP, FAST, SPEC, MK, MULTI>), grid, block, 0, st, a);
             };
diff --git a/pyfilter_amd/filters/particle/base.py b/pyfilter_amd/filters/particle/base.py
--- a/pyfilter_amd/filters/particle/base.py
+++ b/pyfilter_amd/filters/particle/base.py
@@ -5,7 +5,7 @@
 
 from ... import _lib as L
 from ... import ops
-from ...hints import HINTS, ROUTE_AUTO, ROUTE_CLUSTER, ROUTE_PER_STEP
+from ...hints import HINTS, ROUTE_AUTO, ROUTE_CLUSTER, ROUTE_PER_STEP, ROUTE_PER_STEP_GENERIC
 from ...resampling import multinomial, systematic
 from ...timeseries import AffineEulerMaruyama, StateSpaceModel, TimeseriesState
 from ...timeseries.models import pack_params
@@ -393,7 +393,7 @@
     def batch_filter(self, y, bar=True, init_state=None) -> FilterResult:
         return self._batch_filter(y, init_state, bar=bar)[0]
 
-    def _batch_filter(self, y, init_state=None, *, bar=False, defer_status=False, per_step=False):
+    def _batch_filter(self, y, init_state=None, *, bar=False, defer_status=False, per_step=False, generic_steps=False):
         assert self._model is not None, "Model has not been initialized!"
         device, _ = self._device_dtype()
         if (not self._fused_capable(device) or not isinstance(y, torch.Tensor)
@@ -401,8 +401,8 @@
                 or (self._kernel_kind().is_user and FilterResult.states_kept(self.record_states) != 1)):
             return super().batch_filter(y, bar=bar, init_state=init_state), None
         if self._single_launch_run(y):
-            return self._batch_filter_lean(y, init_state, defer_status, per_step)
-        return self._batch_filter_fused(y, init_state), None
+            return self._batch_filter_lean(y, init_state, defer_status, per_step, generic_steps)
+        return self._batch_filter_fused(y, init_state, generic_steps=generic_steps), None
 
     def _single_launch_run(self, y) -> bool:
         return (y.shape[0] > 0 and FilterResult.states_kept(self.record_states) == 1 and not self._time_kernels
@@ -412,10 +412,11 @@
                                             self._resampler_kind() == L.RESAMPLE_SYSTEMATIC))
                 and self._ctx_tapes_none())
 
-    def _batch_filter_lean(self, y: torch.Tensor, init_state, defer_status: bool, per_step: bool):
+    def _batch_filter_lean(self, y: torch.Tensor, init_state, defer_status: bool, per_step: bool, generic_steps: bool = False):
         state = init_state if init_state is not None else self.initialize()
         result = FilterResult(state, self.record_states, self.record_moments, _defer_moments=True)
-        blk, _, _ = self._filter_block_lean(y, state, None, None, host_u=True, defer_status=defer_status, per_step=per_step)
+        blk, _, _ = self._filter_block_lean(y, state, None, None, host_u=True, defer_status=defer_status, per_step=per_step,
+                                            generic_steps=generic_steps)
         result._extend_fused(blk.filter_means, blk.filter_variance, blk.loglikelihood, blk.latest_state)
         self._last_run["rows"] = (blk.filter_means, blk.filter_variance)
         return result, ((blk.status, blk.plan) if blk.status is not None else None)
@@ -503,7 +504,7 @@
         L.check(plan.run(plan.args_ref, t0, n_steps, 1, L.stream_ptr()), "pf_filter_run")
 
     def _filter_block_lean(self, y: torch.Tensor, state: ParticleFilterCorrection, observed, replay, host_u: bool = False,
-                           per_step: bool = False, defer_status: bool = False):
+                           per_step: bool = False, defer_status: bool = False, generic_steps: bool = False):
         ctx = self._ctx
         kind = ctx.kind
         ts_in = state.timeseries_state
@@ -547,7 +548,8 @@
 
         load_state()
         a = plan.args
-        plan.write_hints(None, ROUTE_PER_STEP if per_step else None)
+        per_step = per_step or generic_steps
+        plan.write_hints(None, ROUTE_PER_STEP_GENERIC if generic_steps else (ROUTE_PER_STEP if per_step else None))
         a.model.params = ctx.params.data_ptr()
         a.y, a.y_rows = y_dev.data_ptr(), rows
         a.observed, a.observed_dev = flags.data_ptr(), None
@@ -587,7 +589,7 @@
         res.plan = plan
         return res, ll_steps, (seed_eff, None)
 
-    def _batch_filter_fused(self, y: torch.Tensor, init_state=None, observed=None, replay=None) -> FilterResult:
+    def _batch_filter_fused(self, y: torch.Tensor, init_state=None, observed=None, replay=None, generic_steps: bool = False) -> FilterResult:
         state = init_state if init_state is not None else self.initialize()
         ctx = self._ensure_context()
         kind = ctx.kind
@@ -631,7 +633,7 @@
         use_graph = ((not taped) and not ring and replay is None and not self._time_kernels
                      and HINTS.graph and not kind.is_user and not self._move_by_move)
         key = (n, b, d, o, steps, rows, dtype, device, self._FILTER_KIND, self._proposal._KERNEL_PROPOSAL,
-               self._resampler_kind(), self._seed, float(self._resample_threshold), observed_host.numpy().tobytes(), HINTS.key())
+               self._resampler_kind(), self._seed, float(self._resample_threshold), observed_host.numpy().tobytes(), HINTS.key(), generic_steps)
         user_graph = (kind.is_user and bool(getattr(self._model.hidden, "graph_callable", False)) and (not taped) and not ring
                       and replay is None and not self._time_kernels and HINTS.graph
                       and not isinstance(self._move_by_move, (list, tuple)))
@@ -656,7 +658,7 @@
         word = (seed_eff - self._seed) & _M64
         plan.epoch.fill_(word - (1 << 64) if word >= (1 << 63) else word)
         a = plan.args
-        plan.write_hints(None)
+        plan.write_hints(None, ROUTE_PER_STEP_GENERIC if generic_steps else None)
         z_tape = u_tape = None
         if ctx.z_tape is not None:
             z_tape = ctx.z_tape[t_start:t_start + steps].contiguous()
diff --git a/pyfilter_amd/hints.py b/pyfilter_amd/hints.py
--- a/pyfilter_amd/hints.py
+++ b/pyfilter_amd/hints.py
@@ -1,5 +1,6 @@
 
 ROUTE_AUTO, ROUTE_PER_STEP, ROUTE_COLUMN_GENERIC, ROUTE_CLUSTER, ROUTE_CLUSTER_ALWAYS, ROUTE_CLUSTER_SPREAD = 0, 1, 2, 3, 4, 5
+ROUTE_PER_STEP_GENERIC = 6
 
 
 class RunHints:
diff --git a/pyfilter_amd/ops.py b/pyfilter_amd/ops.py
--- a/pyfilter_amd/ops.py
+++ b/pyfilter_amd/ops.py
@@ -369,7 +369,7 @@
 
 SYNC_CHECKS = False
 
-TRACE_FIELDS = ("step", "tbytes", "D", "VEC", "MODE", "PROP", "FAST", "SPEC", "MK", "MULTI")
+TRACE_FIELDS = ("step", "tbytes", "D", "VEC", "MODE", "PROP", "FAST", "SPEC", "MK", "MULTI", "LEAF")
 
 
 def debug_draw_normals(seed: int, steps: int, n: int, b: int, d: int, dtype, device, step0: int = 0) -> torch.Tensor:
@@ -385,9 +385,9 @@
 
 def debug_launch_trace(last: int = 64):
     buf = (C.c_int32 * (len(TRACE_FIELDS) * last))()
-    n = L.load().pf_debug_launch_trace(buf, last)
+    n = L.load().pf_debug_launch_trace_fields(buf, last, len(TRACE_FIELDS))
     if n < 0:
-        L.check(n, "pf_debug_launch_trace")
+        L.check(n, "pf_debug_launch_trace_fields")
     k = len(TRACE_FIELDS)
     return [dict(zip(TRACE_FIELDS, buf[i * k:(i + 1) * k])) for i in range(n)]
 
```
